# walaj/SeqLib

Hardware: AMD Instinct MI355X
Metric: aligned reads/sec (150 bp) via BWAAligner (higher is better)
Workload: dtype int32

## Files before the change

### seqlib_amd/csrc/dev_chain_coop.h

```cpp
#pragma once
#include "dev_chain.h"

__device__ __forceinline__ int64_t lane_read64(int64_t v, int src)
{
    const int s = __builtin_amdgcn_readfirstlane(src);
    const unsigned lo = (unsigned)__builtin_amdgcn_readlane((int)(v & 0xffffffffll), s);
    const unsigned hi = (unsigned)__builtin_amdgcn_readlane((int)(v >> 32), s);
    return (int64_t)(((unsigned long long)hi << 32) | lo);
}

struct CoopTables {
    int64_t *s_pos;
    int *s_ord;
    int *s_w, *s_cb, *s_ce, *s_first, *s_kept;
    signed char *s_kf;
};

template <typename I, int NCMAX, bool FINAL>
__device__ __noinline__ void dev_chain_read_coop(const DevFM<I> &fm, const DevRef &R, const Chunk &ck, const slx_opt &opt, int r, const CoopTables &T, int lane,
                                                 int nc_limit)
{
    int64_t *s_pos = T.s_pos; int *s_ord = T.s_ord, *s_w = T.s_w, *s_cb = T.s_cb, *s_ce = T.s_ce, *s_first = T.s_first, *s_kept = T.s_kept;
    signed char *s_kf = T.s_kf;
    {
        ReadWS w = make_ws(ck, r);
        const int len = (int)(ck.offs[r + 1] - ck.offs[r]);
        const int n_intv = (int)ck.intv_n[r];
        const qp_t *iinfo = (const qp_t *)ck.intv_info + (size_t)r * ck.cap_intv;
        const I *ix0 = (const I *)ck.intv_x0 + (size_t)r * ck.cap_intv;
        const I *ix2 = (const I *)ck.intv_x2 + (size_t)r * ck.cap_intv;
        int ns = 0, nc = 0;
        bool dup = false;
        KbTree kb;
        bool tree = false;
        int *l_tail = s_w, *l_lastql = s_cb, *l_lastoff = s_ce, *l_firstql = s_first, *l_rid = s_kept;
        const bool cnt16 = ck.seed_off[r + 1] - ck.seed_off[r] < 65536;
        for (int i = 0; i < n_intv; ++i) {
            const int qbeg = QP_HI(iinfo[i]), slen = QP_LO(iinfo[i]) - qbeg;
            const I x0 = ix0[i], x2 = ix2[i];
            const I step = x2 > (I)opt.max_occ ? x2 / (I)opt.max_occ : (I)1;
            I cm = (x2 + step - 1) / step;
            if (cm > (I)opt.max_occ) cm = (I)opt.max_occ;
            const int count_max = (int)cm;
            for (int base = 0; base < count_max; base += 64) {
                const int t = base + lane;
                const bool valid = t < count_max;
                int64_t rb_l = 0; int rid_l = -1;
                if (valid) {
                    rb_l = intv_pos<I>(fm, x0, (I)t * step);
                    rid_l = dev_intv2rid(R, rb_l, rb_l + slen);
                }
                const int nb = count_max - base < 64 ? count_max - base : 64;
                for (int u = 0; u < nb; ++u) {
                    const int rid = __builtin_amdgcn_readlane(rid_l, __builtin_amdgcn_readfirstlane(u));
                    if (rid < 0) continue;
                    const int64_t rbeg = lane_read64(rb_l, u);
                    int lo = -1, lower_c = -1;
                    bool to_add = true;
                    if (nc) {
                        if (tree) lower_c = kb.lower(rbeg);
                        else {
                            int b = 0, e = nc;
                            while (b < e) { const int m = (b + e) >> 1; if (s_pos[m] < rbeg) b = m + 1; else e = m; }
                            if (b == nc) lo = nc - 1;
                            else lo = rbeg < s_pos[b] ? b - 1 : b;
                            lower_c = lo >= 0 ? s_ord[lo] : -1;
                        }
                        if (lower_c >= 0) {
                            const int c = lower_c;
                            const int last = l_tail[c];
#ifdef SLX_WIDE
                            const qp_t lql = w.s_ql[last];
                            const int f_qbeg = w.s_qbeg(w.c_head[c]);
#else
                            const uint32_t lql = (uint32_t)l_lastql[c], fql = (uint32_t)l_firstql[c];
                            const int f_qbeg = (int)(fql >> 16);
#endif
                            const int l_qbeg = QP_HI(lql), l_len = QP_LO(lql);
                            const int64_t f_rbeg = tree ? w.c_pos[c] : s_pos[lo];
                            const int64_t l_rbeg = f_rbeg + l_lastoff[c];
                            const int64_t qend = l_qbeg + l_len, rend = l_rbeg + l_len;
                            int res;
                            if (rid != l_rid[c]) res = 0;
                            else if (qbeg >= f_qbeg && qbeg + slen <= qend && rbeg >= f_rbeg && rbeg + slen <= rend) res = 1;
                            else if ((l_rbeg < R.l_pac || f_rbeg < R.l_pac) && rbeg >= R.l_pac) res = 0;
                            else {
                                const int64_t x = qbeg - l_qbeg, y = rbeg - l_rbeg;
                                if (y >= 0 && x - y <= opt.w && y - x <= opt.w && x - l_len < opt.max_chain_gap && y - l_len < opt.max_chain_gap) {
                                    const int s = ns++;
                                    w.s_rbeg[s] = rbeg; w.s_ql[s] = QP_PACK(qbeg, slen); w.s_next[s] = -1; if (w.s_score) w.s_score[s] = slen;
                                    w.s_next[last] = s; w.c_tail[c] = s;
#ifdef SLX_WIDE
                                    w.c_n[c] = w.c_n[c] + 1;
                                    l_tail[c] = s; l_lastoff[c] = (int)(rbeg - f_rbeg);
#else
                                    if (cnt16) { l_firstql[c] = (int)(fql + 1u); w.c_n[c] = (int)(fql & 0xffff) + 1; }
                                    else w.c_n[c] = w.c_n[c] + 1;
                                    l_tail[c] = s; l_lastql[c] = (int)(((uint32_t)qbeg << 16) | (uint32_t)slen); l_lastoff[c] = (int)(rbeg - f_rbeg);
#endif
                                    res = 1;
                                } else res = 0;
                            }
                            to_add = !res;
                        }
                    }
                    if (to_add && !tree && lo >= 0 && s_pos[lo] == rbeg) dup = true;
                    if (to_add && dup && !tree && nc >= 2 * KB_T - 1) {
                        kb.mem = (int *)w.regs; kb.n_nodes = 0; kb.root = kb.alloc(0);
                        for (int h = 0; h < nc; ++h) kb.put(w.c_pos[h], h);
                        tree = true;
                    }
                    if (to_add && nc == nc_limit) {
                        if (FINAL) { if (lane == 0) dev_chain_read<I>(fm, R, ck, opt, r); }
                        else if (lane == 0) ck.n_chain[r] = -2;
                        return;
                    }
                    if (to_add) {
                        const int s = ns++, c = nc;
                        w.s_rbeg[s] = rbeg; w.s_ql[s] = QP_PACK(qbeg, slen); w.s_next[s] = -1; if (w.s_score) w.s_score[s] = slen;
                        w.c_pos[c] = rbeg; w.c_head[c] = s; w.c_tail[c] = s; w.c_n[c] = 1; w.c_rid[c] = rid;
#ifdef SLX_WIDE
                        l_tail[c] = s; l_lastoff[c] = 0; l_rid[c] = rid;
#else
                        l_tail[c] = s; l_lastql[c] = (int)(((uint32_t)qbeg << 16) | (uint32_t)slen); l_firstql[c] = (int)(((uint32_t)qbeg << 16) | 1u); l_lastoff[c] = 0; l_rid[c] = rid;
#endif
                        if (tree) kb.put(rbeg, c);
                        else {
                            for (int hi = nc; hi > lo + 1; hi -= 64) {
                                const int idx = hi - 1 - lane;
                                const bool mv = idx >= lo + 1;
                                int vo = 0; int64_t vp = 0;
                                if (mv) { vo = s_ord[idx]; vp = s_pos[idx]; }
                                if (mv) { s_ord[idx + 1] = vo; s_pos[idx + 1] = vp; }
                            }
                            s_ord[lo + 1] = c; s_pos[lo + 1] = rbeg;
                        }
                        ++nc;
                    }
                }
            }
        }
        if (tree) kb.traverse(s_ord);
        ck.frac_rep[r] = (float)ck.l_rep[r] / len;
        for (int c = lane; c < nc; c += 64) {
            const int wt = dev_chain_weight(w, c);
            s_w[c] = wt;
            s_cb[c] = w.s_qbeg(w.c_head[c]);
            s_ce[c] = w.s_qbeg(w.c_tail[c]) + w.s_len(w.c_tail[c]);
            s_first[c] = -1; s_kf[c] = 0;
        }
        int n_chn = 0;
        for (int base = 0; base < nc; base += 64) {
            const int m = base + lane;
            int c = 0; bool keep = false;
            if (m < nc) { c = s_ord[m]; keep = s_w[c] >= opt.min_chain_weight; }
            const unsigned long long bal = __ballot(keep);
            const int rank = __popcll(bal & ((1ull << lane) - 1ull));
            if (keep) s_ord[n_chn + rank] = c;
            n_chn += __popcll(bal);
        }
        int n_out = 0;
        if (n_chn > 0) {
            int *a = s_ord;
            ks_introsort_idx(n_chn, a, [&](int x, int y) { return s_w[x] > s_w[y]; });
            int n_kept = 0;
            s_kf[a[0]] = 3;
            s_kept[n_kept++] = 0;
            for (int i = 1; i < n_chn; ++i) {
                const int ci = a[i];
                const int bi = s_cb[ci], ei = s_ce[ci], wi = s_w[ci], li = ei - bi;
                const bool i_alt = ref_is_alt(R, w.c_rid[ci]) != 0;
                int large_ovlp = 0;
                bool broke = false;
                for (int kb = 0; kb < n_kept && !broke; kb += 64) {
                    const int k = kb + lane;
                    bool large = false, drop = false;
                    int cj = 0;
                    if (k < n_kept) {
                        cj = a[s_kept[k]];
                        const int bj = s_cb[cj], ej = s_ce[cj];
                        const int b_max = bj > bi ? bj : bi, e_min = ej < ei ? ej : ei;
                        if (e_min > b_max && (!ref_is_alt(R, w.c_rid[cj]) || i_alt)) {
                            const int lj = ej - bj;
                            const int min_l = li < lj ? li : lj;
                            if ((float)(e_min - b_max) >= (float)min_l * opt.mask_level && min_l < opt.max_chain_gap) {
                                large = true;
                                const int wj = s_w[cj];
                                if ((float)wi < (float)wj * opt.drop_ratio && wj - wi >= opt.min_seed_len << 1) drop = true;
                            }
                        }
                    }
                    const unsigned long long bd = __ballot(drop);
                    const int first_drop = bd ? (int)__ffsll((long long)bd) - 1 : 64;
                    const bool eff = large && lane <= first_drop;
                    if (eff && s_first[cj] < 0) s_first[cj] = i;
                    if (__ballot(eff)) large_ovlp = 1;
                    if (bd) broke = true;
                }
                if (!broke) { s_kept[n_kept++] = i; s_kf[ci] = large_ovlp ? 2 : 3; }
            }
            for (int i = lane; i < n_kept; i += 64) {
                const int c = a[s_kept[i]];
                if (s_first[c] >= 0) s_kf[a[s_first[c]]] = 1;
            }
            int i, k;
            for (i = k = 0; i < n_chn; ++i) {
                const int kf = s_kf[a[i]];
                if (kf == 0 || kf == 3) continue;
                if (++k >= opt.max_chain_extend) break;
            }
            for (int m = i + lane; m < n_chn; m += 64) if (s_kf[a[m]] < 3) s_kf[a[m]] = 0;
            for (int base = 0; base < n_chn; base += 64) {
                const int m = base + lane;
                int c = 0; bool keep = false;
                if (m < n_chn) { c = a[m]; keep = s_kf[c] != 0; }
                const unsigned long long bal = __ballot(keep);
                const int rank = __popcll(bal & ((1ull << lane) - 1ull));
                if (keep) w.ia[n_out + rank] = c;
                n_out += __popcll(bal);
            }
        }
        {
            int carry = 0;
            for (int base = 0; base < n_out; base += 64) {
                const int x = base + lane;
                const int c = x < n_out ? w.ia[x] : 0;
                const int cn = x < n_out ? w.c_n[c] : 0;
                int incl = cn;
                for (int d = 1; d < 64; d <<= 1) { const int t = __shfl_up(incl, d, 64); if (lane >= d) incl += t; }
                if (x < n_out) {
                    int off = carry + incl - cn;
                    w.c_first[c] = off;
                    for (int s = w.c_head[c]; s >= 0; s = w.s_next[s]) w.c_w[off++] = s;
                }
                carry += __shfl(incl, 63, 64);
            }
        }
        if (lane == 0) ck.n_chain[r] = n_out;
    }
}

template <typename I, int NCMAX, bool FINAL>
__global__ void __launch_bounds__(64) k_chain_coop(DevFM<I> fm, DevRef R, Chunk ck, DevOpt dopt, const int *order, unsigned int *queue,
                                                   const unsigned int *n_slots, int nc_limit)
{
    __shared__ int64_t s_pos[NCMAX + 64];
    __shared__ int s_ord[NCMAX + 64];
    __shared__ int s_w[NCMAX], s_cb[NCMAX], s_ce[NCMAX], s_first[NCMAX], s_kept[NCMAX];
    __shared__ signed char s_kf[NCMAX];
    CoopTables T;
    T.s_pos = s_pos; T.s_ord = s_ord; T.s_w = s_w; T.s_cb = s_cb; T.s_ce = s_ce; T.s_first = s_first; T.s_kept = s_kept; T.s_kf = s_kf;
    const int lane = threadIdx.x;
    const int n_todo = __builtin_amdgcn_readfirstlane((int)*n_slots);
    for (;;) {
        const int slot = (int)wave_take(queue, 1u);
        if (slot >= n_todo) break;
        const int r = order ? order[slot] : slot;
        const bool mine = !FINAL || __builtin_amdgcn_readfirstlane(ck.n_chain[r]) == -2;
        if (mine) dev_chain_read_coop<I, NCMAX, FINAL>(fm, R, ck, dopt.o, r, T, lane, nc_limit < NCMAX ? nc_limit : NCMAX);
    }
}
```

### seqlib_amd/csrc/dev_cig_band.h

```cpp
#pragma once
#include "dev_fin2.h"

template <int CPB, typename QF, typename TF>
__device__ int wave_ksw_global2_bandn(int qlen_, QF qf, int tlen_, TF tf, const slx_opt &o, int w_, uint8_t *z, int n_col_, int lane)
{
    const int qlen = __builtin_amdgcn_readfirstlane(qlen_), tlen = __builtin_amdgcn_readfirstlane(tlen_);
    const int w = __builtin_amdgcn_readfirstlane(w_), n_col = __builtin_amdgcn_readfirstlane(n_col_);
    const int o_del = o.o_del, e_del = o.e_del, o_ins = o.o_ins, e_ins = o.e_ins;
    const int oe_del = o_del + e_del, oe_ins = o_ins + e_ins;
    const MatCols mc = make_matcols(o.mat);
    auto pack_of = [&](int j) -> uint32_t {
        const int q = j >= 0 && j < qlen ? qf(j) : 4;
        return q == 0 ? mc.c[0] : q == 1 ? mc.c[1] : q == 2 ? mc.c[2] : q == 3 ? mc.c[3] : mc.c[4];
    };
    const int b0 = lane * CPB;
    int H[CPB], E[CPB];
    uint32_t P[CPB];
#pragma unroll
    for (int c = 0; c < CPB; ++c) {
        const int j = b0 + c - w;
        P[c] = pack_of(j);
        H[c] = j == 0 ? 0 : (j > 0 && j <= qlen && j <= w ? -(o_ins + e_ins * j) : DEV_MINUS_INF);
        E[c] = DEV_MINUS_INF;
    }
    int q_blk = (w + 1) >> 6;
    uint32_t q_cur = pack_of(q_blk * WAVE + lane), q_next = pack_of((q_blk + 1) * WAVE + lane);
    int tb_cur = lane < tlen ? tf(lane) : 0;
    int tb_next = WAVE + lane < tlen ? tf(WAVE + lane) : 0;
#pragma unroll 1
    for (int i = 0; i < tlen; ++i) {
        if ((i & (WAVE - 1)) == 0 && i) { tb_cur = tb_next; tb_next = i + WAVE + lane < tlen ? tf(i + WAVE + lane) : 0; }
        const int t = lane_read(tb_cur, i & (WAVE - 1));
        const uint32_t sh = (uint32_t)t << 3;
        const int beg = i > w ? i - w : 0;
        const int end = i + w + 1 < qlen ? i + w + 1 : qlen;
        const int b_lo = beg - (i - w), b_hi = end - (i - w);
        int m[CPB], exl[CPB];
        bool act[CPB];
        int run = G_NEG;
#pragma unroll
        for (int c = 0; c < CPB; ++c) {
            const int b = b0 + c;
            act[c] = b >= b_lo && b < b_hi;
            m[c] = H[c] + __builtin_amdgcn_sbfe((int)P[c], sh, 8u);
            exl[c] = run;
            const int u = act[c] ? m[c] - oe_ins + b * e_ins : G_NEG;
            run = imax(run, u);
        }
        const int incl = dpp_incl_max_scan_g(run);
        const int lane_ex = dpp_get<0x138, 0xf, 0xf>(G_NEG, incl);
        int e2v[CPB];
#pragma unroll
        for (int c = 0; c < CPB; ++c) {
            const int b = b0 + c;
            const int ex = imax(lane_ex, exl[c]);
            int f = DEV_MINUS_INF - (b - b_lo) * e_ins;
            if (b > b_lo) f = imax(f, ex - (b - 1) * e_ins);
            const int e = E[c];
            int d = m[c] >= e ? 0 : 1;
            int hh = m[c] >= e ? m[c] : e;
            d = hh >= f ? d : 2;
            hh = hh >= f ? hh : f;
            int tt = m[c] - oe_del;
            int e2 = e - e_del;
            d |= e2 > tt ? 1 << 2 : 0;
            e2 = e2 > tt ? e2 : tt;
            tt = m[c] - oe_ins;
            const int f2 = f - e_ins;
            d |= f2 > tt ? 2 << 4 : 0;
            if (act[c] && z) z[(size_t)i * n_col + (b - b_lo)] = (uint8_t)d;
            if (act[c]) H[c] = hh;
            if (b == w - (i + 1)) H[c] = -(o_del + e_del * (i + 1));
            e2v[c] = act[c] ? e2 : DEV_MINUS_INF;
        }
        const int e_in = dpp_get<0x130, 0xf, 0xf>(DEV_MINUS_INF, e2v[0]);
        const uint32_t p_in = (uint32_t)dpp_get<0x130, 0xf, 0xf>(0, (int)P[0]);
        const int jn = i + 1 + w;
        if ((jn >> 6) != q_blk) { q_blk = jn >> 6; q_cur = q_next; q_next = pack_of((q_blk + 1) * WAVE + lane); }
        const uint32_t p_new = jn < qlen ? (uint32_t)lane_read((int)q_cur, jn & (WAVE - 1)) : mc.c[4];
#pragma unroll
        for (int c = 0; c < CPB; ++c) {
            E[c] = c + 1 < CPB ? e2v[c + 1 < CPB ? c + 1 : c] : e_in;
            const uint32_t p_up = c + 1 < CPB ? P[c + 1 < CPB ? c + 1 : c] : p_in;
            P[c] = (b0 + c) == 2 * w ? p_new : p_up;
        }
    }
    const int bf = qlen - 1 - (tlen - 1 - w);
    const int src = bf / CPB, kk = bf - src * CPB;
    int pick = H[0];
#pragma unroll
    for (int c = 1; c < CPB; ++c) pick = kk == c ? H[c] : pick;
    return lane_read(pick, src);
}

#define GB_THREADS 256
#define GB_WAVES (GB_THREADS / WAVE)
struct GbShared { int scan[2][GB_WAVES], edge[2][GB_WAVES]; int result; };

enum { GI_START = 0, GI_NEUTRAL = 1, GI_LOAD = 2 };
struct GRun {
    int i0 = 0, i1 = 0;
    int init = GI_START;
    int rec_row = -1;
    const int *win_in = nullptr;
    int *win_rec = nullptr, *win_out = nullptr;
    int pick = -1;
};

template <int CPB, typename QF, typename TF>
__device__ void block_gband_rows(int qlen, QF qf, int tlen, TF tf, const slx_opt &o, int w, uint8_t *z, int n_col, GbShared &S, const GRun &run)
{
    constexpr int NB = GB_THREADS * CPB;
    const int tid = threadIdx.x, lane = tid & (WAVE - 1), wv = tid >> 6;
    const int o_del = o.o_del, e_del = o.e_del, o_ins = o.o_ins, e_ins = o.e_ins;
    const int oe_del = o_del + e_del, oe_ins = o_ins + e_ins;
    const MatCols mc = make_matcols(o.mat);
    auto pack_of = [&](int j) -> uint32_t {
        const int q = j >= 0 && j < qlen ? qf(j) : 4;
        return q == 0 ? mc.c[0] : q == 1 ? mc.c[1] : q == 2 ? mc.c[2] : q == 3 ? mc.c[3] : mc.c[4];
    };
    const int i0 = run.i0, i1 = run.i1 < tlen ? run.i1 : tlen;
    const int b0 = tid * CPB;
    int H[CPB], E[CPB];
    uint32_t P[CPB];
#pragma unroll
    for (int c = 0; c < CPB; ++c) {
        const int j = i0 + b0 + c - w;
        P[c] = pack_of(j);
        if (run.init == GI_START) { H[c] = j == 0 ? 0 : (j > 0 && j <= qlen && j <= w ? -(o_ins + e_ins * j) : DEV_MINUS_INF); E[c] = DEV_MINUS_INF; }
        else if (run.init == GI_NEUTRAL) { H[c] = 0; E[c] = DEV_MINUS_INF; }
        else { H[c] = run.win_in[b0 + c]; E[c] = run.win_in[NB + b0 + c]; }
    }
    const int top = (wv + 1) * WAVE * CPB;
    int q_blk = (i0 + top - w) >> 6;
    uint32_t q_cur = pack_of(q_blk * WAVE + lane), q_next = pack_of((q_blk + 1) * WAVE + lane);
    const int tb0 = i0 & ~(WAVE - 1);
    int tb_cur = tb0 + lane < tlen ? tf(tb0 + lane) : 0;
    int tb_next = tb0 + WAVE + lane < tlen ? tf(tb0 + WAVE + lane) : 0;
    __syncthreads();
#pragma unroll 1
    for (int i = i0; i < i1; ++i) {
        const int par = i & 1;
        if ((i & (WAVE - 1)) == 0 && i > i0) { tb_cur = tb_next; tb_next = i + WAVE + lane < tlen ? tf(i + WAVE + lane) : 0; }
        const int t = lane_read(tb_cur, i & (WAVE - 1));
        const uint32_t sh = (uint32_t)t << 3;
        const int beg = i > w ? i - w : 0;
        const int end = i + w + 1 < qlen ? i + w + 1 : qlen;
        const int b_lo = beg - (i - w), b_hi = end - (i - w);
        int m[CPB], exl[CPB];
        bool act[CPB];
        int run_u = G_NEG;
#pragma unroll
        for (int c = 0; c < CPB; ++c) {
            const int b = b0 + c;
            act[c] = b >= b_lo && b < b_hi;
            m[c] = H[c] + __builtin_amdgcn_sbfe((int)P[c], sh, 8u);
            exl[c] = run_u;
            const int u = act[c] ? m[c] - oe_ins + b * e_ins : G_NEG;
            run_u = imax(run_u, u);
        }
        const int incl = dpp_incl_max_scan_g(run_u);
        int lane_ex = dpp_get<0x138, 0xf, 0xf>(G_NEG, incl);
        if (lane == WAVE - 1) S.scan[par][wv] = incl;
        __syncthreads();
        if (i > i0 && lane == WAVE - 1 && wv < GB_WAVES - 1) E[CPB - 1] = S.edge[par ^ 1][wv + 1];
        if (i == run.rec_row) {
#pragma unroll
            for (int c = 0; c < CPB; ++c) { run.win_rec[b0 + c] = H[c]; run.win_rec[NB + b0 + c] = E[c]; }
        }
        uint8_t *zr = (z && i >= run.rec_row) ? z : nullptr;
#pragma unroll
        for (int k = 0; k < GB_WAVES - 1; ++k) { const int v = S.scan[par][k]; if (k < wv) lane_ex = imax(lane_ex, v); }
        int e2v[CPB];
#pragma unroll
        for (int c = 0; c < CPB; ++c) {
            const int b = b0 + c;
            const int ex = imax(lane_ex, exl[c]);
            int f = DEV_MINUS_INF - (b - b_lo) * e_ins;
            if (b > b_lo) f = imax(f, ex - (b - 1) * e_ins);
            const int e = E[c];
            int d = m[c] >= e ? 0 : 1;
            int hh = m[c] >= e ? m[c] : e;
            d = hh >= f ? d : 2;
            hh = hh >= f ? hh : f;
            int tt = m[c] - oe_del;
            int e2 = e - e_del;
            d |= e2 > tt ? 1 << 2 : 0;
            e2 = e2 > tt ? e2 : tt;
            tt = m[c] - oe_ins;
            const int f2 = f - e_ins;
            d |= f2 > tt ? 2 << 4 : 0;
            if (act[c] && zr) zr[(size_t)i * n_col + (b - b_lo)] = (uint8_t)d;
            if (act[c]) H[c] = hh;
            if (b == w - (i + 1)) H[c] = -(o_del + e_del * (i + 1));
            e2v[c] = act[c] ? e2 : DEV_MINUS_INF;
        }
        if (lane == 0) S.edge[par][wv] = e2v[0];
        const int e_in = dpp_get<0x130, 0xf, 0xf>(DEV_MINUS_INF, e2v[0]);
        const uint32_t p_in = (uint32_t)dpp_get<0x130, 0xf, 0xf>(0, (int)P[0]);
        const int jn = i - w + top;
        if ((jn >> 6) != q_blk) { q_blk = jn >> 6; q_cur = q_next; q_next = pack_of((q_blk + 1) * WAVE + lane); }
        const uint32_t p_top = (uint32_t)lane_read((int)q_cur, jn & (WAVE - 1));
#pragma unroll
        for (int c = 0; c < CPB; ++c) {
            E[c] = c + 1 < CPB ? e2v[c + 1 < CPB ? c + 1 : c] : e_in;
            const uint32_t p_up = c + 1 < CPB ? P[c + 1 < CPB ? c + 1 : c] : p_in;
            P[c] = (c == CPB - 1 && lane == WAVE - 1) ? p_top : p_up;
        }
    }
    if (run.win_out) {
        __syncthreads();
        if (i1 > i0 && lane == WAVE - 1 && wv < GB_WAVES - 1) E[CPB - 1] = S.edge[(i1 - 1) & 1][wv + 1];
#pragma unroll
        for (int c = 0; c < CPB; ++c) { run.win_out[b0 + c] = H[c]; run.win_out[NB + b0 + c] = E[c]; }
    }
    if (run.pick >= 0) {
#pragma unroll
        for (int c = 0; c < CPB; ++c) if (b0 + c == run.pick) S.result = H[c];
        __syncthreads();
    }
}

template <int CPB, typename QF, typename TF>
__device__ int block_ksw_global2_bandn(int qlen, QF qf, int tlen, TF tf, const slx_opt &o, int w, uint8_t *z, int n_col, GbShared &S)
{
    GRun run;
    run.i0 = 0; run.i1 = tlen; run.init = GI_START;
    run.pick = qlen - 1 - (tlen - 1 - w);
    block_gband_rows<CPB>(qlen, qf, tlen, tf, o, w, z, n_col, S, run);
    return S.result;
}

#define CIG_BAND_MAX_COLS (13 * WAVE)

struct CigBlockShared { GbShared gb; unsigned long long off; int n_ops_dummy; };
struct GJob;
struct GPlan;
struct CigSeg { const GPlan *P = nullptr; const GJob *gj = nullptr; unsigned int job_t = 0; int *scratch = nullptr; };
template <typename QF, typename TF>
__device__ int gseg_join_any(int lq, QF qf, int rlen, TF tf, const slx_opt &o, const CigSeg &cs, uint8_t *z, GbShared &S);
__device__ bool gseg_is_cut(const CigSeg &cs, int ww, int n_col, unsigned long long *z_off);

template <bool BLOCK>
static __device__ __noinline__ bool dev_cig_band_job(const DevRef &R, const Chunk &ck, const slx_opt &opt, const FinLists &fl, uint32_t slot, int lane, CigBlockShared *SB = nullptr,
                                                     const CigSeg *cs = nullptr)
{
    [[maybe_unused]] const bool wave0 = !BLOCK || threadIdx.x < WAVE;
    const DJob j = fl.jobs[slot];
    DHit h = ck.hits[slot];
    const uint8_t *query = ck.codes + ck.offs[j.r];
    const int l_query = (int)(ck.offs[j.r + 1] - ck.offs[j.r]);
    const int lq = j.qe - j.qb;
    const int64_t rb = j.rb, re = j.re;
    const uint8_t *qseg = query + j.qb;
    const bool valid = !(lq <= 0 || rb >= re || (rb < R.l_pac && re > R.l_pac));
    const int rlen = (int)(re - rb);
    const bool rev = rb >= R.l_pac;
    auto qf = [&](int x) { return (int)(rev ? qseg[lq - 1 - x] : qseg[x]); };
    auto tf = [&](int y) { return rev ? ref_base(R, re - 1 - y) : ref_base(R, rb + y); };
    int w2 = j.w2, score = 0, last_sc = -(1 << 30), w_used = 0, n_col = 0;
    uint8_t *z = nullptr;
    if (valid) {
        for (int it = 0; it < 3; ++it) {
            w2 = w2 < opt.w << 2 ? w2 : opt.w << 2;
            int ww, max_gap, max_ins, max_del, min_w;
            max_ins = (int)((double)(((lq + 1) >> 1) * opt.mat[0] - opt.o_ins) / opt.e_ins + 1.);
            max_del = (int)((double)(((lq + 1) >> 1) * opt.mat[0] - opt.o_del) / opt.e_del + 1.);
            max_gap = max_ins > max_del ? max_ins : max_del;
            max_gap = max_gap > 1 ? max_gap : 1;
            const int dl = rlen - lq < 0 ? lq - rlen : rlen - lq;
            ww = (max_gap + dl + 1) >> 1;
            ww = ww < w2 ? ww : w2;
            min_w = dl + 3;
            ww = ww > min_w ? ww : min_w;
            w_used = ww;
            n_col = lq < 2 * ww + 1 ? lq : 2 * ww + 1;
            if (2 * ww + 1 > CIG_BAND_MAX_COLS) return false;
            const unsigned long long need = (unsigned long long)n_col * (unsigned long long)rlen;
            unsigned long long off = 0;
            if constexpr (BLOCK) {
                unsigned long long z_off = 0;
                if (it == 0 && cs && gseg_is_cut(*cs, ww, n_col, &z_off)) {
                    z = ck.zarena + z_off;
                    score = gseg_join_any(lq, qf, rlen, tf, opt, *cs, z, SB->gb);
                    if (score == last_sc || w2 == opt.w << 2) break;
                    last_sc = score;
                    w2 <<= 1;
                    if (!(score < j.truesc - opt.a)) break;
                    continue;
                }
                __syncthreads();
                if (block_tid() == 0) SB->off = atomicAdd(ck.zused, need);
                __syncthreads();
                off = SB->off;
            } else off = wave_take_u64(ck.zused, need);
            if (off + need > ck.zcap) { if (lane == 0 && wave0) atomicOr(ck.flags, OVF_ZARENA | (BLOCK ? OVS_Z_BAND_BLOCK : OVS_Z_BAND)); return true; }
            z = ck.zarena + off;
            const int cols = 2 * ww + 1;
            if constexpr (BLOCK) {
                if (cols <= GB_THREADS) score = block_ksw_global2_bandn<1>(lq, qf, rlen, tf, opt, ww, z, n_col, SB->gb);
                else if (cols <= 2 * GB_THREADS) score = block_ksw_global2_bandn<2>(lq, qf, rlen, tf, opt, ww, z, n_col, SB->gb);
                else score = block_ksw_global2_bandn<4>(lq, qf, rlen, tf, opt, ww, z, n_col, SB->gb);
            } else
            if (cols <= WAVE) score = wave_ksw_global2_bandn<1>(lq, qf, rlen, tf, opt, ww, z, n_col, lane);
            else if (cols <= 2 * WAVE) score = wave_ksw_global2_bandn<2>(lq, qf, rlen, tf, opt, ww, z, n_col, lane);
            else if (cols <= 4 * WAVE) score = wave_ksw_global2_bandn<4>(lq, qf, rlen, tf, opt, ww, z, n_col, lane);
            else if (cols <= 8 * WAVE) score = wave_ksw_global2_bandn<8>(lq, qf, rlen, tf, opt, ww, z, n_col, lane);
            else score = wave_ksw_global2_bandn<13>(lq, qf, rlen, tf, opt, ww, z, n_col, lane);
            if (score == last_sc || w2 == opt.w << 2) break;
            last_sc = score;
            w2 <<= 1;
            if (!(score < j.truesc - opt.a)) break;
        }
    }
    if constexpr (BLOCK) {
        __threadfence();
        __syncthreads();
        if (!wave0) return true;
    }
    int n_ops = 0;
    if (valid) {
        __threadfence();
        dev_traceback_wave(z, n_col, lq, rlen, w_used, lane, [&](int, int) { ++n_ops; });
    }
    n_ops = __builtin_amdgcn_readfirstlane(n_ops);
    const unsigned long long need = (unsigned long long)n_ops + 2;
    const unsigned long long base = wave_take_u64(ck.cigused, need);
    if (base + need > ck.cigcap) { if (lane == 0) atomicOr(ck.flags, OVF_CIGAR | OVS_C_BAND); return true; }
    uint32_t *cg = ck.cigpool + base + 1;
    if (valid) {
        int wp = n_ops;
        dev_traceback_wave(z, n_col, lq, rlen, w_used, lane, [&](int op, int len) { cg[--wp] = (uint32_t)len << 4 | (uint32_t)op; });
        int x = 0, y = 0, n_mm = 0, n_gap = 0;
        for (int k = 0; k < n_ops; ++k) {
            const uint32_t cw = cg[k];
            const int op = (int)(cw & 0xf), len = (int)(cw >> 4);
            if (op == 0) {
                for (int u = lane; u < len; u += WAVE) n_mm += qf(x + u) != tf(y + u);
                x += len; y += len;
            } else if (op == 2) { if (k > 0 && k < n_ops - 1) n_gap += len; y += len; }
            else if (op == 1) { x += len; n_gap += len; }
        }
        for (int d = 32; d >= 1; d >>= 1) n_mm += __shfl_xor(n_mm, d, WAVE);
        h.nm = n_mm + n_gap;
    }
    dev_finish_hit(R, ck, j, l_query, h, (int64_t)base + 1, n_ops);
    if (lane == 0) ck.hits[slot] = h;
    return true;
}

__global__ void __launch_bounds__(64) k_cig_band(DevRef R, Chunk ck, DevOpt dopt, FinLists fl, uint32_t *rest, unsigned int *n_rest)
{
    const int lane = threadIdx.x;
    const unsigned int n_jobs = *fl.n_dp;
    for (;;) {
        const unsigned int t = wave_take(fl.q_dp, 1u);
        if (t >= n_jobs) break;
        const uint32_t slot = fl.dp_list[t];
        if (!dev_cig_band_job<false>(R, ck, dopt.o, fl, slot, lane) && lane == 0) rest[atomicAdd(n_rest, 1u)] = slot;
    }
}


struct RegsBlockShared {
    GbShared gb;
    int cmd, w, l_query, rlen, rev;
    const uint8_t *qseg;
    int64_t rb, re;
};

__device__ __noinline__ int regs_block_dp(const DevRef &R, const slx_opt &o, RegsBlockShared &S)
{
    const int w = S.w, l_query = S.l_query, rlen = S.rlen;
    const bool rev = S.rev != 0;
    const uint8_t *qseg = S.qseg;
    const int64_t rb = S.rb, re = S.re;
    auto qf = [&](int x) { return (int)(rev ? qseg[l_query - 1 - x] : qseg[x]); };
    auto tf = [&](int y) { return rev ? ref_base(R, re - 1 - y) : ref_base(R, rb + y); };
    const int cols = 2 * w + 1;
    if (cols <= GB_THREADS) return block_ksw_global2_bandn<1>(l_query, qf, rlen, tf, o, w, nullptr, 0, S.gb);
    if (cols <= 2 * GB_THREADS) return block_ksw_global2_bandn<2>(l_query, qf, rlen, tf, o, w, nullptr, 0, S.gb);
    return block_ksw_global2_bandn<4>(l_query, qf, rlen, tf, o, w, nullptr, 0, S.gb);
}

struct PMemo { const GJob *jobs; const int *off, *n; };
__device__ bool pseg_lookup(const PMemo *pm, int r, int w_arg, unsigned long long q_off, int l_query, int64_t rb, int64_t re, int *score);

#ifdef PSEG_DEBUG
__device__ void pseg_debug_miss(const PMemo *pm, int r, int w_arg, unsigned long long q_off, int l_query, int64_t rb, int64_t re);
#endif
struct WaveScorerLong {
    const DevRef &R; const slx_opt &o; const Chunk &ck; int lane; int *eh_h, *eh_e;
    RegsBlockShared *SB;
    const PMemo *pm = nullptr;
    const int *cur_r = nullptr;
    __device__ int operator()(int w_, int l_query, const uint8_t *qseg, int64_t rb, int64_t re) const
    {
        if (l_query <= 0 || rb >= re || (rb < R.l_pac && re > R.l_pac)) return 0;
        if (pm) { int ms = 0; if (pseg_lookup(pm, *cur_r, w_, (unsigned long long)(qseg - ck.codes), l_query, rb, re, &ms)) return ms; }
#ifdef PSEG_DEBUG
        if (pm && lane == 0 && re - rb >= 16384) pseg_debug_miss(pm, *cur_r, w_, (unsigned long long)(qseg - ck.codes), l_query, rb, re);
#endif
        const int rlen = (int)(re - rb);
        const bool rev = rb >= R.l_pac;
        auto qf = [&](int x) { return (int)(rev ? qseg[l_query - 1 - x] : qseg[x]); };
        auto tf = [&](int y) { return rev ? ref_base(R, re - 1 - y) : ref_base(R, rb + y); };
        if (l_query == rlen && w_ == 0) {
            int sc = 0;
            for (int i = lane; i < l_query; i += WAVE) sc += o.mat[tf(i) * 5 + qf(i)];
            for (int d = 32; d >= 1; d >>= 1) sc += __shfl_xor(sc, d, WAVE);
            return sc;
        }
        int max_ins = (int)((double)(((l_query + 1) >> 1) * o.mat[0] - o.o_ins) / o.e_ins + 1.);
        int max_del = (int)((double)(((l_query + 1) >> 1) * o.mat[0] - o.o_del) / o.e_del + 1.);
        int max_gap = max_ins > max_del ? max_ins : max_del;
        max_gap = max_gap > 1 ? max_gap : 1;
        const int dl = rlen - l_query < 0 ? l_query - rlen : rlen - l_query;
        int w = (max_gap + dl + 1) >> 1;
        w = w < w_ ? w : w_;
        const int min_w = dl + 3;
        w = w > min_w ? w : min_w;
        const int cols = 2 * w + 1;
        if (SB && cols > 2 * WAVE && cols <= 4 * GB_THREADS && rlen >= 2048) {
            if (lane == 0) { SB->w = w; SB->l_query = l_query; SB->rlen = rlen; SB->rev = rev ? 1 : 0; SB->qseg = qseg; SB->rb = rb; SB->re = re; SB->cmd = 1; }
            __syncthreads();
            return regs_block_dp(R, o, *SB);
        }
        if (cols <= WAVE) return wave_ksw_global2_bandn<1>(l_query, qf, rlen, tf, o, w, nullptr, 0, lane);
        if (cols <= 2 * WAVE) return wave_ksw_global2_bandn<2>(l_query, qf, rlen, tf, o, w, nullptr, 0, lane);
        if (cols <= 4 * WAVE) return wave_ksw_global2_bandn<4>(l_query, qf, rlen, tf, o, w, nullptr, 0, lane);
        if (cols <= 8 * WAVE) return wave_ksw_global2_bandn<8>(l_query, qf, rlen, tf, o, w, nullptr, 0, lane);
        if (cols <= CIG_BAND_MAX_COLS) return wave_ksw_global2_bandn<13>(l_query, qf, rlen, tf, o, w, nullptr, 0, lane);
        int sc = 0;
        if (lane == 0) sc = dev_gen_cigar2<0>(R, o, ck, w_, l_query, qseg, rb, re, false, eh_h, eh_e).score;
        return lane_read(sc, 0);
    }
};

template <int MAXQ, int NB>
__global__ void __launch_bounds__(GB_THREADS) k_regs_wave_long(DevRef R, Chunk ck, DevOpt dopt, FinLists fl, const int *order, unsigned int *queue, const unsigned int *n_slots,
                                                               PMemo pm)
{
    __shared__ int s_idx[NB], s_ka[NB], s_kb[NB], s_qe[NB], s_rid[NB], s_w[NB];
    __shared__ int64_t s_k64[NB], s_rb[NB];
    __shared__ RegsBlockShared SB;
    if ((int)blockIdx.x * WAVE >= ck.long_threads) return;
    if (threadIdx.x >= WAVE) {
        for (;;) {
            __syncthreads();
            if (SB.cmd == 0) break;
            regs_block_dp(R, dopt.o, SB);
        }
        return;
    }
    const int lane = threadIdx.x;
    SortStage ss;
    ss.idx = s_idx; ss.k64 = s_k64; ss.ka = s_ka; ss.kb = s_kb; ss.m_rb = s_rb; ss.m_qe = s_qe; ss.m_rid = s_rid; ss.m_w = s_w;
    ss.nmax = NB; ss.lane = lane;
    int *eh_h = ck.long_scratch + (size_t)blockIdx.x * WAVE * 2 * ck.long_stride, *eh_e = eh_h + ck.long_stride;
    int cur_r = 0;
    WaveScorerLong sc{R, dopt.o, ck, lane, eh_h, eh_e, &SB, pm.jobs ? &pm : nullptr, &cur_r};
    const int n_todo = __builtin_amdgcn_readfirstlane((int)*n_slots);
    for (;;) {
        const int slot = (int)wave_take(queue, 1u);
        if (slot >= n_todo) break;
        const int r = order ? order[slot] : slot;
        cur_r = r;
        dev_regs_read<MAXQ>(R, ck, dopt.o, fl, r, sc, lane == 0, &ss);
    }
    if (lane == 0) SB.cmd = 0;
    __syncthreads();
}
```

### seqlib_amd/csrc/dev_fin.h

```cpp
#pragma once
#include "dev_ext.h"

#define DEV_MINUS_INF (-0x40000000)

template <typename QF, typename TF>
__device__ int dev_ksw_global2(int qlen, QF qf, int tlen, TF tf, const slx_opt &o, int w, uint8_t *z, int n_col, int *eh_h, int *eh_e)
{
    const int8_t *mat = o.mat;
    const int o_del = o.o_del, e_del = o.e_del, o_ins = o.o_ins, e_ins = o.e_ins;
    const int oe_del = o_del + e_del, oe_ins = o_ins + e_ins;
    int i, j;
    eh_h[0] = 0; eh_e[0] = DEV_MINUS_INF;
    for (j = 1; j <= qlen && j <= w; ++j) { eh_h[j] = -(o_ins + e_ins * j); eh_e[j] = DEV_MINUS_INF; }
    for (; j <= qlen; ++j) eh_h[j] = eh_e[j] = DEV_MINUS_INF;
    for (i = 0; i < tlen; ++i) {
        int f = DEV_MINUS_INF, h1, beg, end, t;
        const int8_t *qrow = mat + tf(i) * 5;
        beg = i > w ? i - w : 0;
        end = i + w + 1 < qlen ? i + w + 1 : qlen;
        h1 = beg == 0 ? -(o_del + e_del * (i + 1)) : DEV_MINUS_INF;
        uint8_t *zi = z ? z + (size_t)i * n_col : nullptr;
        for (j = beg; j < end; ++j) {
            int h, m = eh_h[j], e = eh_e[j];
            uint8_t d;
            eh_h[j] = h1;
            m += qrow[qf(j)];
            d = m >= e ? 0 : 1;
            h = m >= e ? m : e;
            d = h >= f ? d : 2;
            h = h >= f ? h : f;
            h1 = h;
            t = m - oe_del;
            e -= e_del;
            d |= e > t ? 1 << 2 : 0;
            e = e > t ? e : t;
            eh_e[j] = e;
            t = m - oe_ins;
            f -= e_ins;
            d |= f > t ? 2 << 4 : 0;
            f = f > t ? f : t;
            if (zi) zi[j - beg] = d;
        }
        eh_h[end] = h1; eh_e[end] = DEV_MINUS_INF;
    }
    return eh_h[qlen];
}

template <typename ZAT, typename F>
__device__ void dev_traceback_at(ZAT zat, int qlen, int tlen, int w, F emit)
{
    int i = tlen - 1, k = (i + w + 1 < qlen ? i + w + 1 : qlen) - 1, which = 0;
    int cur_op = -1, cur_len = 0;
    auto unit = [&](int op, int len) {
        if (op == cur_op) cur_len += len;
        else { if (cur_op >= 0) emit(cur_op, cur_len); cur_op = op; cur_len = len; }
    };
    while (i >= 0 && k >= 0) {
        which = zat(i, k - (i > w ? i - w : 0)) >> (which << 1) & 3;
        if (which == 0) { unit(0, 1); --i; --k; }
        else if (which == 1) { unit(2, 1); --i; }
        else { unit(1, 1); --k; }
    }
    if (i >= 0) unit(2, i + 1);
    if (k >= 0) unit(1, k + 1);
    if (cur_op >= 0) emit(cur_op, cur_len);
}
template <typename F>
__device__ void dev_traceback(const uint8_t *z, int n_col, int qlen, int tlen, int w, F emit)
{
    dev_traceback_at([&](int i, int c) { return (int)z[(size_t)i * n_col + c]; }, qlen, tlen, w, emit);
}

struct GenCig {
    int score;
    bool valid;
    bool fast;
    bool rev;
    int w, n_col, qlen, tlen;
    uint8_t *z;
};

template <int MAXQ>
__device__ GenCig dev_gen_cigar2(const DevRef &R, const slx_opt &o, const Chunk &ck, int w_, int l_query, const uint8_t *qseg,
                                 int64_t rb, int64_t re, bool want_z, int *eh_h, int *eh_e)
{
    GenCig g;
    g.score = 0; g.valid = false; g.fast = false; g.rev = false; g.w = 0; g.n_col = 0; g.qlen = l_query; g.tlen = 0; g.z = nullptr;
    if (l_query <= 0 || rb >= re || (rb < R.l_pac && re > R.l_pac)) return g;
    g.valid = true;
    const int rlen = (int)(re - rb);
    g.tlen = rlen;
    g.rev = rb >= R.l_pac;
    const bool rev = g.rev;
    auto qf = [&](int j) { return (int)(rev ? qseg[l_query - 1 - j] : qseg[j]); };
    auto tf = [&](int i) { return rev ? ref_base(R, re - 1 - i) : ref_base(R, rb + i); };
    if (l_query == rlen && w_ == 0) {
        g.fast = true;
        int sc = 0;
        for (int i = 0; i < l_query; ++i) sc += o.mat[tf(i) * 5 + qf(i)];
        g.score = sc;
    } else {
        int w, max_gap, max_ins, max_del, min_w;
        max_ins = (int)((double)(((l_query + 1) >> 1) * o.mat[0] - o.o_ins) / o.e_ins + 1.);
        max_del = (int)((double)(((l_query + 1) >> 1) * o.mat[0] - o.o_del) / o.e_del + 1.);
        max_gap = max_ins > max_del ? max_ins : max_del;
        max_gap = max_gap > 1 ? max_gap : 1;
        const int dl = rlen - l_query < 0 ? l_query - rlen : rlen - l_query;
        w = (max_gap + dl + 1) >> 1;
        w = w < w_ ? w : w_;
        min_w = dl + 3;
        w = w > min_w ? w : min_w;
        g.w = w;
        g.n_col = l_query < 2 * w + 1 ? l_query : 2 * w + 1;
        if (want_z) {
            const unsigned long long need = (unsigned long long)g.n_col * (unsigned long long)rlen;
            const unsigned long long off = atomicAdd(ck.zused, need);
            if (off + need > ck.zcap) { atomicOr(ck.flags, OVF_ZARENA | OVS_Z_GEN); g.valid = false; return g; }
            g.z = ck.zarena + off;
        }
        g.score = dev_ksw_global2(l_query, qf, rlen, tf, o, w, g.z, g.n_col, eh_h, eh_e);
    }
    return g;
}

__device__ __forceinline__ int dev_patch_pre(const DevRef &R, const slx_opt &o, int64_t a_rb, int64_t a_re, int a_qb, int a_qe, int a_w,
                                             int64_t b_rb, int64_t b_re, int b_qb, int b_qe, int b_w)
{
    int w;
    double r;
    if (a_rb < R.l_pac && b_rb >= R.l_pac) return -1;
    if (a_qb >= b_qb || a_qe >= b_qe || a_re >= b_re) return -1;
    w = (int)((a_re - b_rb) - (a_qe - b_qb));
    w = w > 0 ? w : -w;
    r = (double)(a_re - b_rb) / (double)(b_re - a_rb) - (double)(a_qe - b_qb) / (double)(b_qe - a_qb);
    r = r > 0. ? r : -r;
    if (a_re < b_rb || a_qe < b_qb) {
        if (w > o.w << 1 || r >= (double)0.05f) return -1;
    } else if (w > o.w << 2 || r >= (double)(0.05f * 2)) return -1;
    w += a_w + b_w;
    w = w < o.w << 2 ? w : o.w << 2;
    return w;
}

template <int MAXQ, typename SC>
__device__ int dev_patch_reg(const DevRef &R, const slx_opt &o, const Chunk &ck, const uint8_t *query, const DReg &a, const DReg &b,
                             int *_w, SC &sc)
{
    int score, q_s, r_s;
    const int w = dev_patch_pre(R, o, a.rb, a.re, a.qb, a.qe, a.w, b.rb, b.re, b.qb, b.qe, b.w);
    if (w < 0) return 0;
    score = sc(w, b.qe - a.qb, query + a.qb, a.rb, b.re);
    q_s = (int)((double)(b.qe - a.qb) / (double)((b.qe - b.qb) + (a.qe - a.qb)) * (double)(b.score + a.score) + .499);
    r_s = (int)((double)(b.re - a.rb) / (double)((b.re - b.rb) + (a.re - a.rb)) * (double)(b.score + a.score) + .499);
    if ((double)score / (double)(q_s > r_s ? q_s : r_s) < (double)0.90f) return 0;
    *_w = w;
    return score;
}

__device__ __forceinline__ uint64_t dev_hash_64(uint64_t key)
{
    key += ~(key << 32); key ^= (key >> 22); key += ~(key << 13); key ^= (key >> 8);
    key += (key << 3); key ^= (key >> 15); key += ~(key << 27); key ^= (key >> 31);
    return key;
}

__device__ __forceinline__ uint64_t dev_lrand48_nth(uint64_t state, uint64_t n)
{
    const uint64_t M = (1ULL << 48) - 1;
    uint64_t a = 0x5DEECE66DULL, c = 0xBULL, ra = 1, rc = 0;
    while (n) {
        if (n & 1) { ra = (ra * a) & M; rc = (rc * a + c) & M; }
        c = ((a + 1) * c) & M;
        a = (a * a) & M;
        n >>= 1;
    }
    return ((ra * (state & M) + rc) & M) >> 17;
}

__device__ __forceinline__ int dev_infer_bw(int l1, int l2, int score, int a, int q, int r)
{
    int w;
    if (l1 == l2 && l1 * a - score < (q + r - a) << 1) return 0;
    w = (int)((double)((l1 < l2 ? l1 : l2) * a - score - q) / r + 2.);
    const int d = l1 - l2 < 0 ? l2 - l1 : l1 - l2;
    if (w < d) w = d;
    return w;
}

__device__ inline int dev_approx_mapq_se(const slx_opt &o, const DReg &a, const Chunk &ck)
{
    int mapq, l, sub = a.sub ? a.sub : o.min_seed_len * o.a;
    double identity;
    sub = a.csub > sub ? a.csub : sub;
    if (sub >= a.score) return 0;
    l = a.qe - a.qb > a.re - a.rb ? a.qe - a.qb : (int)(a.re - a.rb);
    identity = 1. - (double)(l * o.a - a.score) / (double)(o.a + o.b) / (double)l;
    if (a.score == 0) mapq = 0;
    else if (o.mapQ_coef_len > 0) {
        double tmp;
        if ((float)l < o.mapQ_coef_len) tmp = 1.;
        else {
            if (l >= ck.log_lut_n) { atomicOr(ck.flags, ERR_LOGLUT); return 0; }
            tmp = (double)o.mapQ_coef_fac / ck.log_lut[l];
        }
        tmp *= identity * identity;
        mapq = (int)(6.02 * (double)(a.score - sub) / (double)o.a * tmp * tmp + .499);
    } else {
        if (a.seedcov >= ck.log_lut_n || a.seedcov < 1) { atomicOr(ck.flags, ERR_LOGLUT); return 0; }
        mapq = (int)(30.0 * (1. - (double)sub / (double)a.score) * ck.log_lut[a.seedcov] + .499);
        mapq = identity < 0.95 ? (int)((double)mapq * identity * identity + .499) : mapq;
    }
    if (a.sub_n > 0) {
        if (a.sub_n + 1 >= ck.log_lut_n) { atomicOr(ck.flags, ERR_LOGLUT); return 0; }
        mapq -= (int)(4.343 * ck.log_lut[a.sub_n + 1] + .499);
    }
    if (mapq > 60) mapq = 60;
    if (mapq < 0) mapq = 0;
    mapq = (int)((double)mapq * (1. - (double)a.frac_rep) + .499);
    return mapq;
}

__device__ inline void dev_mark_primary_alt(const DevRef &R, const slx_opt &opt, const ReadWS &w, int n, uint64_t id)
{
    int *a = w.ia, *z = w.ib;
    int *par = (int *)w.srt;
    DReg *G = w.regs;
    auto alt = [&](int h) { return ref_is_alt(R, G[h].rid); };
    int tmp = opt.a + opt.b;
    tmp = opt.o_del + opt.e_del > tmp ? opt.o_del + opt.e_del : tmp;
    tmp = opt.o_ins + opt.e_ins > tmp ? opt.o_ins + opt.e_ins : tmp;
    auto core = [&](int m) {
        int nz = 0;
        z[nz++] = 0;
        for (int i = 1; i < m; ++i) {
            int k;
            DReg &ai = G[a[i]];
            for (k = 0; k < nz; ++k) {
                DReg &aj = G[a[z[k]]];
                const int b_max = aj.qb > ai.qb ? aj.qb : ai.qb;
                const int e_min = aj.qe < ai.qe ? aj.qe : ai.qe;
                if (e_min > b_max) {
                    const int min_l = ai.qe - ai.qb < aj.qe - aj.qb ? ai.qe - ai.qb : aj.qe - aj.qb;
                    if ((float)(e_min - b_max) >= (float)min_l * opt.mask_level) {
                        if (aj.sub == 0) aj.sub = ai.score;
                        if (aj.score - ai.score <= tmp && (alt(a[z[k]]) || !alt(a[i]))) ++aj.sub_n;
                        break;
                    }
                }
            }
            if (k == nz) z[nz++] = i;
            else ai.secondary = z[k];
        }
    };
    int n_pri = 0;
    for (int i = 0; i < n; ++i) {
        DReg &p = G[a[i]];
        p.sub = 0; p.secondary = -1;
        p.hash = dev_hash_64(id + (uint64_t)i);
        if (!alt(a[i])) ++n_pri;
    }
    ks_introsort_idx(n, a, [&](int x, int y) {
        const DReg &X = G[x], &Y = G[y];
        if (X.score != Y.score) return X.score > Y.score;
        const int ax = alt(x), ay = alt(y);
        return ax < ay || (ax == ay && X.hash < Y.hash);
    });
    core(n);
    if (n_pri < n) {
        for (int i = 0; i < n; ++i) { const int sidx = G[a[i]].secondary; par[a[i]] = sidx >= 0 ? a[sidx] : -1; }
        if (n_pri > 0)
            ks_introsort_idx(n, a, [&](int x, int y) {
                const DReg &X = G[x], &Y = G[y];
                const int ax = alt(x), ay = alt(y);
                if (ax != ay) return ax < ay;
                return X.score > Y.score || (X.score == Y.score && X.hash < Y.hash);
            });
        for (int i = 0; i < n; ++i) z[a[i]] = i;
        for (int i = 0; i < n; ++i) {
            const int h = a[i], ph = par[h];
            if (ph >= 0) { par[h] = z[ph]; if (alt(h)) G[h].secondary = 0x7fffffff; }
            else par[h] = -1;
        }
        if (n_pri > 0) {
            for (int i = 0; i < n_pri; ++i) { DReg &p = G[a[i]]; p.sub = 0; p.secondary = -1; }
            core(n_pri);
        }
    } else
        for (int i = 0; i < n; ++i) par[a[i]] = G[a[i]].secondary;
}

struct SortStage {
    int *idx;
    int64_t *k64;
    int *ka, *kb;
    int64_t *m_rb;
    int *m_qe, *m_rid, *m_w;
    int nmax;
    int lane;
};

template <int MAXQ>
__device__ __forceinline__ void fin_sync()
{
    if constexpr (MAXQ > 704) { __builtin_amdgcn_fence(__ATOMIC_ACQ_REL, "workgroup"); __builtin_amdgcn_wave_barrier(); }
    else __syncthreads();
}

template <int MAXQ, typename SC>
__device__ int dev_fin_regs(const DevRef &R, const Chunk &ck, const slx_opt &opt, ReadWS &w, int r, const uint8_t *query, int l_query, SC &sc,
                            const SortStage *ss = nullptr, bool *defer = nullptr)
{
        int n = ck.n_reg[r];
        int *a = w.ia;
        DReg *G = w.regs;
        const bool staged = ss != nullptr && n <= ss->nmax && n >= 2;
        const bool dbg = ck.dbg_cyc && ck.dbg_stage == 2;
        unsigned long long t0 = dbg ? __builtin_readcyclecounter() : 0ull, t1 = t0, t2 = t0, t3 = t0;
        auto sort_handles = [&](int m, auto fill, auto less_lds, auto less_glb) {
            if (!staged) { ks_introsort_idx(m, a, less_glb); return; }
            __threadfence_block();
            for (int i = ss->lane; i < m; i += 64) { const int h = a[i]; ss->idx[i] = h; fill(h); }
            fin_sync<MAXQ>();
            bool tie = m > 768;
            if (!tie) for (int e = ss->lane; e < m; e += 64) {
                const int he = ss->idx[e];
                int rank = 0;
                for (int j = 0; j < m; ++j) {
                    const int hj = ss->idx[j];
                    const bool lt = less_lds(hj, he);
                    rank += lt ? 1 : 0;
                    if (!lt && j != e && !less_lds(he, hj)) tie = true;
                }
                ss->m_w[e] = rank;
            }
            if (!__any(tie)) {
                fin_sync<MAXQ>();
                for (int e = ss->lane; e < m; e += 64) ss->m_rid[ss->m_w[e]] = ss->idx[e];
                fin_sync<MAXQ>();
                for (int e = ss->lane; e < m; e += 64) { const int h = ss->m_rid[e]; ss->idx[e] = h; a[e] = h; }
            } else {
                fin_sync<MAXQ>();
                if (ss->lane == 0) ks_introsort_idx(m, ss->idx, less_lds);
                fin_sync<MAXQ>();
                for (int i = ss->lane; i < m; i += 64) a[i] = ss->idx[i];
            }
            fin_sync<MAXQ>();
            __threadfence_block();
        };
        if (staged) { for (int i = ss->lane; i < n; i += 64) a[i] = i; __threadfence_block(); }
        else for (int i = 0; i < n; ++i) a[i] = i;
        if (n > 1) {
            sort_handles(n, [&](int h) { ss->k64[h] = G[h].re; },
                         [&](int x, int y) { return ss->k64[x] < ss->k64[y]; },
                         [&](int x, int y) { return G[x].re < G[y].re; });
            if (dbg) t1 = __builtin_readcyclecounter();
            if (defer && !staged && n <= 64) {
                for (int i = 1; i < n; ++i) {
                    const DReg &p = G[a[i]];
                    if (p.rid != G[a[i - 1]].rid || p.rb >= G[a[i - 1]].re + opt.max_chain_gap) continue;
                    for (int j = i - 1; j >= 0 && p.rid == G[a[j]].rid && p.rb < G[a[j]].re + opt.max_chain_gap; --j) {
                        const DReg &q = G[a[j]];
                        if (q.rb < p.rb && dev_patch_pre(R, opt, q.rb, q.re, q.qb, q.qe, q.w, p.rb, p.re, p.qb, p.qe, p.w) >= 0) { *defer = true; return -1; }
                    }
                }
            }
            if (staged) { for (int i = ss->lane; i < n; i += 64) G[i].n_comp = 1; __threadfence_block(); }
            else for (int i = 0; i < n; ++i) G[a[i]].n_comp = 1;
            if (staged) {
                const int lane = ss->lane;
                int64_t *m_re = ss->k64; int *m_sc = ss->ka, *m_qb = ss->kb;
                for (int h = lane; h < n; h += 64) {
                    const DReg &g = G[h];
                    ss->m_rb[h] = g.rb; m_re[h] = g.re; m_qb[h] = g.qb; ss->m_qe[h] = g.qe; ss->m_rid[h] = g.rid; m_sc[h] = g.score; ss->m_w[h] = g.w;
                }
                fin_sync<MAXQ>();
                for (int i = 1; i < n; ++i) {
                    const int ph = ss->idx[i], prevh = ss->idx[i - 1];
                    if (ss->m_rid[ph] != ss->m_rid[prevh] || ss->m_rb[ph] >= m_re[prevh] + opt.max_chain_gap) continue;
                    int jtop = i - 1;
                    while (jtop >= 0) {
                        const int64_t p_rb = ss->m_rb[ph], p_re = m_re[ph];
                        const int p_qb = m_qb[ph], p_qe = ss->m_qe[ph], p_rid = ss->m_rid[ph], p_sc = m_sc[ph], p_w = ss->m_w[ph];
                        const int j = jtop - lane;
                        const bool valid = j >= 0;
                        const int qh = ss->idx[valid ? j : 0];
                        const int64_t q_rb = ss->m_rb[qh], q_re = m_re[qh];
                        const int q_qb = m_qb[qh], q_qe = ss->m_qe[qh], q_sc = m_sc[qh], q_w = ss->m_w[qh];
                        const bool cond = valid && p_rid == ss->m_rid[qh] && p_rb < q_re + opt.max_chain_gap;
                        const unsigned long long stopm = __ballot(!cond);
                        const int first_stop = stopm ? (int)__ffsll((long long)stopm) - 1 : 64;
                        const bool live = lane < first_stop;
                        int cat = 0;
                        if (live && q_qe != q_qb) {
                            const int64_t orr = q_re - p_rb;
                            const int64_t oq = q_qb < p_qb ? q_qe - p_qb : p_qe - q_qb;
                            const int64_t mr = q_re - q_rb < p_re - p_rb ? q_re - q_rb : p_re - p_rb;
                            const int64_t mq = q_qe - q_qb < p_qe - p_qb ? q_qe - q_qb : p_qe - p_qb;
                            if ((float)orr > opt.mask_level_redun * (float)mr && (float)oq > opt.mask_level_redun * (float)mq) cat = p_sc < q_sc ? 2 : 1;
                            else if (q_rb < p_rb && dev_patch_pre(R, opt, q_rb, q_re, q_qb, q_qe, q_w, p_rb, p_re, p_qb, p_qe, p_w) >= 0) cat = 3;
                        }
                        const unsigned long long evm = __ballot(cat >= 2);
                        const int first_ev = evm ? (int)__ffsll((long long)evm) - 1 : 64;
                        if (cat == 1 && lane < first_ev) { ss->m_qe[qh] = q_qb; G[qh].qe = q_qb; }
                        fin_sync<MAXQ>();
                        if (first_ev == 64) {
                            if (first_stop < 64) break;
                            jtop -= 64;
                            continue;
                        }
                        const int ev_cat = __builtin_amdgcn_readlane(cat, first_ev);
                        const int ev_q = __builtin_amdgcn_readlane(qh, first_ev);
                        if (ev_cat == 2) {
                            if (lane == 0) { ss->m_qe[ph] = p_qb; G[ph].qe = p_qb; }
                            fin_sync<MAXQ>();
                            break;
                        }
                        {
                            DReg &pp = G[ph];
                            DReg &q = G[ev_q];
                            int ww = 0;
                            const int score = dev_patch_reg<MAXQ>(R, opt, ck, query, q, pp, &ww, sc);
                            if (score > 0) {
                                pp.n_comp += q.n_comp + 1;
                                pp.seedcov = pp.seedcov > q.seedcov ? pp.seedcov : q.seedcov;
                                pp.sub = pp.sub > q.sub ? pp.sub : q.sub;
                                pp.csub = pp.csub > q.csub ? pp.csub : q.csub;
                                pp.qb = q.qb; pp.rb = q.rb;
                                pp.truesc = pp.score = score;
                                pp.w = ww;
                                q.qb = q.qe;
                                if (lane == 0) {
                                    m_qb[ph] = m_qb[ev_q]; ss->m_rb[ph] = ss->m_rb[ev_q]; m_sc[ph] = score; ss->m_w[ph] = ww;
                                    m_qb[ev_q] = ss->m_qe[ev_q];
                                }
                                fin_sync<MAXQ>();
                            }
                        }
                        jtop -= first_ev + 1;
                    }
                }
                __threadfence_block();
            } else
            for (int i = 1; i < n; ++i) {
                DReg &p = G[a[i]];
                if (p.rid != G[a[i - 1]].rid || p.rb >= G[a[i - 1]].re + opt.max_chain_gap) continue;
                for (int j = i - 1; j >= 0 && p.rid == G[a[j]].rid && p.rb < G[a[j]].re + opt.max_chain_gap; --j) {
                    DReg &q = G[a[j]];
                    int64_t orr, oq, mr, mq;
                    int score, ww;
                    if (q.qe == q.qb) continue;
                    orr = q.re - p.rb;
                    oq = q.qb < p.qb ? q.qe - p.qb : p.qe - q.qb;
                    mr = q.re - q.rb < p.re - p.rb ? q.re - q.rb : p.re - p.rb;
                    mq = q.qe - q.qb < p.qe - p.qb ? q.qe - q.qb : p.qe - p.qb;
                    if ((float)orr > opt.mask_level_redun * (float)mr && (float)oq > opt.mask_level_redun * (float)mq) {
                        if (p.score < q.score) { p.qe = p.qb; break; }
                        else q.qe = q.qb;
                    } else if (q.rb < p.rb && (score = dev_patch_reg<MAXQ>(R, opt, ck, query, q, p, &ww, sc)) > 0) {
                        p.n_comp += q.n_comp + 1;
                        p.seedcov = p.seedcov > q.seedcov ? p.seedcov : q.seedcov;
                        p.sub = p.sub > q.sub ? p.sub : q.sub;
                        p.csub = p.csub > q.csub ? p.csub : q.csub;
                        p.qb = q.qb; p.rb = q.rb;
                        p.truesc = p.score = score;
                        p.w = ww;
                        q.qb = q.qe;
                    }
                }
            }
            if (dbg) t2 = __builtin_readcyclecounter();
            auto compact_staged = [&](int n_in, int first_forced) {
                int m = 0;
                for (int base = 0; base < n_in; base += 64) {
                    const int i = base + ss->lane;
                    const int h = i < n_in ? ss->idx[i] : 0;
                    const bool keep = i < n_in && (i < first_forced || ss->m_qe[h] > ss->kb[h]);
                    const unsigned long long km = __ballot(keep);
                    const int pos = m + (int)__builtin_amdgcn_mbcnt_hi((uint32_t)(km >> 32), __builtin_amdgcn_mbcnt_lo((uint32_t)km, 0u));
                    if (keep) a[pos] = h;
                    m += (int)__popcll(km);
                }
                __threadfence_block();
                return m;
            };
            int m = 0;
            if (staged) m = compact_staged(n, 0);
            else for (int i = 0; i < n; ++i) if (G[a[i]].qe > G[a[i]].qb) a[m++] = a[i];
            n = m;
            sort_handles(n, [&](int h) { ss->ka[h] = G[h].score; ss->k64[h] = G[h].rb; ss->kb[h] = G[h].qb; },
                         [&](int x, int y) {
                             const int sx = ss->ka[x], sy = ss->ka[y];
                             const int64_t bx = ss->k64[x], by = ss->k64[y];
                             return sx > sy || (sx == sy && (bx < by || (bx == by && ss->kb[x] < ss->kb[y])));
                         },
                         [&](int x, int y) {
                             const DReg &X = G[x], &Y = G[y];
                             return X.score > Y.score || (X.score == Y.score && (X.rb < Y.rb || (X.rb == Y.rb && X.qb < Y.qb)));
                         });
            if (staged) {
                for (int i = 1 + ss->lane; i < n; i += 64) {
                    const int h = ss->idx[i], hp = ss->idx[i - 1];
                    if (ss->ka[h] == ss->ka[hp] && ss->k64[h] == ss->k64[hp] && ss->kb[h] == ss->kb[hp]) { G[h].qe = ss->kb[h]; ss->m_qe[h] = ss->kb[h]; }
                }
                fin_sync<MAXQ>();
                n = compact_staged(n, 1);
            } else {
                for (int i = 1; i < n; ++i)
                    if (G[a[i]].score == G[a[i - 1]].score && G[a[i]].rb == G[a[i - 1]].rb && G[a[i]].qb == G[a[i - 1]].qb)
                        G[a[i]].qe = G[a[i]].qb;
                m = n > 0 ? 1 : 0;
                for (int i = 1; i < n; ++i) if (G[a[i]].qe > G[a[i]].qb) a[m++] = a[i];
                n = m;
            }
        }
        if (dbg) t3 = __builtin_readcyclecounter();
        ck.na[r] = n;
        if (n > 0) {
            const uint64_t id = dev_lrand48_nth(ck.rng_state, ck.first_ordinal + (uint64_t)r + 1);
            int tmp = opt.a + opt.b;
            tmp = opt.o_del + opt.e_del > tmp ? opt.o_del + opt.e_del : tmp;
            tmp = opt.o_ins + opt.e_ins > tmp ? opt.o_ins + opt.e_ins : tmp;
            auto core_staged = [&](int m, const int *l_alt) {
                const int lane = ss->lane;
                int *l_sub = ss->m_rid, *l_subn = ss->m_w, *l_sec = (int *)ss->k64, *l_z = (int *)ss->k64 + ss->nmax;
                fin_sync<MAXQ>();
                for (int i = lane; i < m; i += 64) { const int h = ss->idx[i]; l_sub[h] = 0; l_subn[h] = G[h].sub_n; l_sec[h] = -1; }
                if (lane == 0) l_z[0] = 0;
                fin_sync<MAXQ>();
                int nz = 1;
                for (int i = 1; i < m; ++i) {
                    const int hi = ss->idx[i];
                    const int i_qb = ss->kb[hi], i_qe = ss->m_qe[hi], i_sc = ss->ka[hi];
                    int found = -1;
                    for (int kb0 = 0; kb0 < nz && found < 0; kb0 += 64) {
                        const int k = kb0 + lane;
                        bool hit = false;
                        if (k < nz) {
                            const int hj = ss->idx[l_z[k]];
                            const int j_qb = ss->kb[hj], j_qe = ss->m_qe[hj];
                            const int b_max = j_qb > i_qb ? j_qb : i_qb;
                            const int e_min = j_qe < i_qe ? j_qe : i_qe;
                            if (e_min > b_max) {
                                const int min_l = i_qe - i_qb < j_qe - j_qb ? i_qe - i_qb : j_qe - j_qb;
                                hit = (float)(e_min - b_max) >= (float)min_l * opt.mask_level;
                            }
                        }
                        const unsigned long long hm = __ballot(hit);
                        if (hm) found = kb0 + (int)__ffsll((long long)hm) - 1;
                    }
                    if (found >= 0) {
                        if (lane == 0) {
                            const int zi = l_z[found];
                            const int hj = ss->idx[zi];
                            if (l_sub[hj] == 0) l_sub[hj] = i_sc;
                            if (ss->ka[hj] - i_sc <= tmp && (!l_alt || l_alt[hj] || !l_alt[hi])) ++l_subn[hj];
                            l_sec[hi] = zi;
                        }
                    } else { if (lane == 0) l_z[nz] = i; ++nz; }
                    fin_sync<MAXQ>();
                }
                for (int i = lane; i < m; i += 64) { const int h = ss->idx[i]; DReg &p = G[h]; p.sub = l_sub[h]; p.sub_n = l_subn[h]; p.secondary = l_sec[h]; }
                __threadfence_block();
                fin_sync<MAXQ>();
            };
            if (R.ann_alt && staged) {
                const int lane = ss->lane;
                int *l_alt = (int *)ss->m_rb, *l_par = (int *)ss->m_rb + ss->nmax, *par = (int *)w.srt;
                fin_sync<MAXQ>();
                int n_pri = 0;
                for (int base = 0; base < n; base += 64) {
                    const int i = base + lane;
                    bool pri = false;
                    if (i < n) {
                        const int h = a[i];
                        DReg &p = G[h];
                        p.sub = 0; p.secondary = -1; p.hash = dev_hash_64(id + (uint64_t)i);
                        const int al = ref_is_alt(R, p.rid);
                        l_alt[h] = al;
                        pri = !al;
                    }
                    n_pri += (int)__popcll(__ballot(pri));
                }
                __threadfence_block();
                sort_handles(n, [&](int h) { ss->ka[h] = G[h].score; ss->k64[h] = (int64_t)G[h].hash; },
                             [&](int x, int y) {
                                 const int sx = ss->ka[x], sy = ss->ka[y];
                                 if (sx != sy) return sx > sy;
                                 const int ax = l_alt[x], ay = l_alt[y];
                                 return ax < ay || (ax == ay && (uint64_t)ss->k64[x] < (uint64_t)ss->k64[y]);
                             },
                             [&](int x, int y) { return false; });
                core_staged(n, l_alt);
                if (n_pri < n) {
                    for (int i = lane; i < n; i += 64) { const int h = ss->idx[i], sidx = G[h].secondary; l_par[h] = sidx >= 0 ? ss->idx[sidx] : -1; }
                    fin_sync<MAXQ>();
                    if (n_pri > 0)
                        sort_handles(n, [&](int h) { ss->ka[h] = G[h].score; ss->k64[h] = (int64_t)G[h].hash; },
                                     [&](int x, int y) {
                                         const int ax = l_alt[x], ay = l_alt[y];
                                         if (ax != ay) return ax < ay;
                                         const int sx = ss->ka[x], sy = ss->ka[y];
                                         return sx > sy || (sx == sy && (uint64_t)ss->k64[x] < (uint64_t)ss->k64[y]);
                                     },
                                     [&](int x, int y) { return false; });
                    int *l_rank = (int *)ss->k64;
                    fin_sync<MAXQ>();
                    for (int i = lane; i < n; i += 64) l_rank[ss->idx[i]] = i;
                    fin_sync<MAXQ>();
                    for (int i = lane; i < n; i += 64) {
                        const int h = ss->idx[i], ph = l_par[h];
                        if (ph >= 0) { par[h] = l_rank[ph]; if (l_alt[h]) G[h].secondary = 0x7fffffff; }
                        else par[h] = -1;
                    }
                    if (n_pri > 0) {
                        __threadfence_block();
                        core_staged(n_pri, l_alt);
                    }
                } else
                    for (int i = lane; i < n; i += 64) { const int h = ss->idx[i]; par[h] = G[h].secondary; }
                __threadfence_block();
                fin_sync<MAXQ>();
            } else if (R.ann_alt) {
                dev_mark_primary_alt(R, opt, w, n, id);
            } else {
            if (staged) {
                for (int i = ss->lane; i < n; i += 64) { DReg &p = G[a[i]]; p.sub = 0; p.secondary = -1; p.hash = dev_hash_64(id + (uint64_t)i); }
                __threadfence_block();
            } else for (int i = 0; i < n; ++i) {
                DReg &p = G[a[i]];
                p.sub = 0; p.secondary = -1;
                p.hash = dev_hash_64(id + (uint64_t)i);
            }
            sort_handles(n, [&](int h) { ss->ka[h] = G[h].score; ss->k64[h] = (int64_t)G[h].hash; },
                         [&](int x, int y) {
                             const int sx = ss->ka[x], sy = ss->ka[y];
                             return sx > sy || (sx == sy && (uint64_t)ss->k64[x] < (uint64_t)ss->k64[y]);
                         },
                         [&](int x, int y) {
                             const DReg &X = G[x], &Y = G[y];
                             return X.score > Y.score || (X.score == Y.score && X.hash < Y.hash);
                         });
            if (staged) core_staged(n, nullptr);
            else {
            int *z = w.ib, nz = 0;
            z[nz++] = 0;
            for (int i = 1; i < n; ++i) {
                int k;
                DReg &ai = G[a[i]];
                for (k = 0; k < nz; ++k) {
                    DReg &aj = G[a[z[k]]];
                    const int b_max = aj.qb > ai.qb ? aj.qb : ai.qb;
                    const int e_min = aj.qe < ai.qe ? aj.qe : ai.qe;
                    if (e_min > b_max) {
                        const int min_l = ai.qe - ai.qb < aj.qe - aj.qb ? ai.qe - ai.qb : aj.qe - aj.qb;
                        if ((float)(e_min - b_max) >= (float)min_l * opt.mask_level) {
                            if (aj.sub == 0) aj.sub = ai.score;
                            if (aj.score - ai.score <= tmp) ++aj.sub_n;
                            break;
                        }
                    }
                }
                if (k == nz) z[nz++] = i;
                else ai.secondary = z[k];
            }
            }
            }
        }
        if (dbg) {
            const unsigned long long t4 = __builtin_readcyclecounter();
            ck.dbg_cyc[r] = t4 - t0; ck.dbg_cyc[(size_t)ck.n_reads + r] = t1 - t0; ck.dbg_cyc[2 * (size_t)ck.n_reads + r] = t2 - t1;
            ck.dbg_cyc[3 * (size_t)ck.n_reads + r] = t3 - t2;
        }
        return n;
}


struct HitsSoA {
    int64_t *hit_off; int32_t *rid; int64_t *pos; uint16_t *flag; uint8_t *mapq; int32_t *score, *nm, *na, *n_cigar_ops;
    int64_t *cig_off; uint32_t *cigar;
    int32_t *xa_parent, *sub;
};

__global__ void k_hit_counts(Chunk ck, unsigned long long *n_cig_words)
{
    const int r = blockIdx.x * blockDim.x + threadIdx.x;
    if (r >= ck.n_reads) return;
    const uint64_t o = ck.seed_off[r];
    unsigned long long c = 0;
    for (int i = 0; i < ck.n_hit[r]; ++i) c += (unsigned long long)ck.hits[o + ck.ic[o + i]].n_cigar;
    n_cig_words[r] = c;
}

__global__ void k_compact(Chunk ck, const unsigned long long *hit_off, const unsigned long long *cig_off_read, HitsSoA out,
                          int64_t read_base, int64_t hit_base, int64_t cig_base)
{
    const int r = blockIdx.x * blockDim.x + threadIdx.x;
    if (r >= ck.n_reads) return;
    const uint64_t o = ck.seed_off[r];
    int64_t ho = hit_base + (int64_t)hit_off[r];
    int64_t co = cig_base + (int64_t)cig_off_read[r];
    out.hit_off[read_base + r] = ho;
    for (int i = 0; i < ck.n_hit[r]; ++i, ++ho) {
        const DHit &h = ck.hits[o + ck.ic[o + i]];
        out.rid[ho] = h.rid; out.pos[ho] = h.pos; out.flag[ho] = (uint16_t)h.flag; out.mapq[ho] = (uint8_t)h.mapq;
        if (out.xa_parent) {
            out.xa_parent[ho] = ((h.flag >> 16) & 0x7fff) - 1;
            const DReg &g = ck.regs[o + ck.ia[o + ck.ic[o + i]]];
            out.sub[ho] = h.flag < 0 ? (g.sub > g.csub ? g.sub : g.csub) : -1;
        }
        out.score[ho] = h.score; out.nm[ho] = h.nm; out.na[ho] = ck.na[r]; out.n_cigar_ops[ho] = h.n_cigar;
        out.cig_off[ho] = co;
        for (int k = 0; k < h.n_cigar; ++k) out.cigar[co++] = ck.cigpool[h.cig_start + k];
    }
}
```

### seqlib_amd/csrc/dev_fin2.h

```cpp
#pragma once
#include "dev_fin.h"
#include "dev_ext_reg.h"
#include "dev_nm8.h"

#ifndef LANE_CIG_BAND
#define LANE_CIG_BAND 33
#endif
#define LANE_CIG_MAXQ 158
#define LANE_CIG_MAXT 400
#define LANE_NEG (-16000)
#define LANE_FIN_LIMIT 8000
static_assert(LANE_NEG + LANE_FIN_LIMIT <= -LANE_FIN_LIMIT && LANE_NEG >= -32768 && LANE_FIN_LIMIT <= 32767, "16-bit cells of k_cig_lanes");
#define LANE_IL_WORDS(max_len) (((LANE_CIG_BAND + 3) / 4) * (((max_len) < LANE_CIG_MAXQ ? (max_len) : LANE_CIG_MAXQ) + 16))
struct alignas(8) DJob {
    int64_t rb, re;
    int qb, qe;
    int w2, truesc;
    int r, pad;
};

struct FinLists {
    DJob *jobs;
    uint32_t *fast_list, *dp_list;
    unsigned int *n_fast, *n_dp, *q_dp;
    uint32_t *lane_list;
    unsigned int *n_lane;
};

#define G_NEG ((int)0x80000000)

__device__ __forceinline__ int dpp_incl_max_scan_g(int v)
{
    v = imax(v, dpp_get<0x111, 0xf, 0xf>(G_NEG, v));
    v = imax(v, dpp_get<0x112, 0xf, 0xf>(G_NEG, v));
    v = imax(v, dpp_get<0x114, 0xf, 0xf>(G_NEG, v));
    v = imax(v, dpp_get<0x118, 0xf, 0xf>(G_NEG, v));
    v = imax(v, dpp_get<0x142, 0xa, 0xf>(G_NEG, v));
    v = imax(v, dpp_get<0x143, 0xc, 0xf>(G_NEG, v));
    return v;
}

template <int CPL, typename QF, typename TF>
__device__ int wave_ksw_global2(int qlen_, QF qf, int tlen_, TF tf, const slx_opt &o, const MatRows &mr, int w_, uint8_t *z, int n_col_, int lane)
{
    const int qlen = __builtin_amdgcn_readfirstlane(qlen_), tlen = __builtin_amdgcn_readfirstlane(tlen_);
    const int w = __builtin_amdgcn_readfirstlane(w_), n_col = __builtin_amdgcn_readfirstlane(n_col_);
    const int o_del = o.o_del, e_del = o.e_del, o_ins = o.o_ins, e_ins = o.e_ins;
    const int oe_del = o_del + e_del, oe_ins = o_ins + e_ins;
    const int j0 = lane * CPL;
    const MatCols mc = make_matcols(o.mat);
    int H[CPL], E[CPL];
    uint32_t P[CPL];
#pragma unroll
    for (int k = 0; k < CPL; ++k) {
        const int j = j0 + k;
        const int q = j < qlen ? qf(j) : 4;
        P[k] = q == 0 ? mc.c[0] : q == 1 ? mc.c[1] : q == 2 ? mc.c[2] : q == 3 ? mc.c[3] : mc.c[4];
        H[k] = j == 0 ? 0 : (j <= qlen && j <= w ? -(o_ins + e_ins * j) : DEV_MINUS_INF);
        E[k] = DEV_MINUS_INF;
    }
    int tb_cur = lane < tlen ? tf(lane) : 0;
    int tb_next = WAVE + lane < tlen ? tf(WAVE + lane) : 0;
#ifdef CIG_NOUNROLL
#pragma unroll 1
#endif
    for (int i = 0; i < tlen; ++i) {
        if ((i & (WAVE - 1)) == 0 && i) { tb_cur = tb_next; tb_next = i + WAVE + lane < tlen ? tf(i + WAVE + lane) : 0; }
        const int t = lane_read(tb_cur, i & (WAVE - 1));
        const uint32_t sh = (uint32_t)t << 3;
        const int beg = i > w ? i - w : 0;
        const int end = i + w + 1 < qlen ? i + w + 1 : qlen;
        const int h1_init = beg == 0 ? -(o_del + e_del * (i + 1)) : DEV_MINUS_INF;
        int M[CPL], pre[CPL], h[CPL];
        int run = G_NEG;
#pragma unroll
        for (int k = 0; k < CPL; ++k) {
            const int j = j0 + k;
            const bool act = j >= beg && j < end;
            const int s = __builtin_amdgcn_sbfe((int)P[k], sh, 8u);
            M[k] = H[k] + s;
            const int u = act ? M[k] - oe_ins + j * e_ins : G_NEG;
            run = imax(run, u);
            pre[k] = run;
        }
        const int incl = dpp_incl_max_scan_g(run);
        const int excl = dpp_get<0x138, 0xf, 0xf>(G_NEG, incl);
        uint8_t *zi = z ? z + (size_t)i * n_col : nullptr;
#pragma unroll
        for (int k = 0; k < CPL; ++k) {
            const int j = j0 + k;
            const bool act = j >= beg && j < end;
            const int ex = k == 0 ? excl : imax(excl, pre[k - 1]);
            int f = DEV_MINUS_INF - (j - beg) * e_ins;
            if (j > beg) f = imax(f, ex - (j - 1) * e_ins);
            const int m = M[k], e = E[k];
            int d = m >= e ? 0 : 1;
            int hh = m >= e ? m : e;
            d = hh >= f ? d : 2;
            hh = hh >= f ? hh : f;
            h[k] = hh;
            int tt = m - oe_del;
            int e2 = e - e_del;
            d |= e2 > tt ? 1 << 2 : 0;
            e2 = e2 > tt ? e2 : tt;
            tt = m - oe_ins;
            const int f2 = f - e_ins;
            d |= f2 > tt ? 2 << 4 : 0;
            if (act) { E[k] = e2; if (zi) zi[j - beg] = (uint8_t)d; }
        }
        const int h_left = dpp_get<0x138, 0xf, 0xf>(0, h[CPL - 1]);
#pragma unroll
        for (int k = 0; k < CPL; ++k) {
            const int j = j0 + k;
            const int hp = k == 0 ? h_left : h[k - 1];
            if (j - 1 >= beg && j - 1 < end) H[k] = hp;
            if (end > beg) { if (j == beg) H[k] = h1_init; if (j == end) E[k] = DEV_MINUS_INF; }
            else if (j == end) { H[k] = h1_init; E[k] = DEV_MINUS_INF; }
        }
    }
    const int src = qlen / CPL, kk = qlen - src * CPL;
    int pick = H[0];
#pragma unroll
    for (int k = 1; k < CPL; ++k) pick = kk == k ? H[k] : pick;
    return lane_read(pick, src);
}

template <int NCH, typename QF, typename TF>
__device__ int wave_ksw_global2_band(int qlen_, QF qf, int tlen_, TF tf, const slx_opt &o, int w_, uint8_t *z, int n_col_, int lane)
{
    const int qlen = __builtin_amdgcn_readfirstlane(qlen_), tlen = __builtin_amdgcn_readfirstlane(tlen_);
    const int w = __builtin_amdgcn_readfirstlane(w_), n_col = __builtin_amdgcn_readfirstlane(n_col_);
    const int o_del = o.o_del, e_del = o.e_del, o_ins = o.o_ins, e_ins = o.e_ins;
    const int oe_del = o_del + e_del, oe_ins = o_ins + e_ins;
    const MatCols mc = make_matcols(o.mat);
    auto pack_of = [&](int j) -> uint32_t {
        const int q = j >= 0 && j < qlen ? qf(j) : 4;
        return q == 0 ? mc.c[0] : q == 1 ? mc.c[1] : q == 2 ? mc.c[2] : q == 3 ? mc.c[3] : mc.c[4];
    };
    uint32_t Pblk[NCH];
#pragma unroll
    for (int c = 0; c < NCH; ++c) Pblk[c] = pack_of(c * WAVE + lane);
    const int b = lane, bE = b * e_ins;
    uint32_t P = pack_of(b - w);
    int H, E = DEV_MINUS_INF;
    {
        const int j = b - w;
        H = j == 0 ? 0 : (j > 0 && j <= qlen && j <= w ? -(o_ins + e_ins * j) : DEV_MINUS_INF);
    }
    int tb_cur = lane < tlen ? tf(lane) : 0;
    int tb_next = WAVE + lane < tlen ? tf(WAVE + lane) : 0;
#ifdef CIG_NOUNROLL
#pragma unroll 1
#endif
    for (int i = 0; i < tlen; ++i) {
        if ((i & (WAVE - 1)) == 0 && i) { tb_cur = tb_next; tb_next = i + WAVE + lane < tlen ? tf(i + WAVE + lane) : 0; }
        const int t = lane_read(tb_cur, i & (WAVE - 1));
        const uint32_t sh = (uint32_t)t << 3;
        const int beg = i > w ? i - w : 0;
        const int end = i + w + 1 < qlen ? i + w + 1 : qlen;
        const int b_lo = beg - (i - w), b_hi = end - (i - w);
        const bool act = b >= b_lo && b < b_hi;
        const int s = __builtin_amdgcn_sbfe((int)P, sh, 8u);
        const int m = H + s;
        const int u = act ? m - oe_ins + bE : G_NEG;
        const int incl = dpp_incl_max_scan_g(u);
        const int ex = dpp_get<0x138, 0xf, 0xf>(G_NEG, incl);
        int f = DEV_MINUS_INF - (b - b_lo) * e_ins;
        if (b > b_lo) f = imax(f, ex - (b - 1) * e_ins);
        const int e = E;
        int d = m >= e ? 0 : 1;
        int hh = m >= e ? m : e;
        d = hh >= f ? d : 2;
        hh = hh >= f ? hh : f;
        int tt = m - oe_del;
        int e2 = e - e_del;
        d |= e2 > tt ? 1 << 2 : 0;
        e2 = e2 > tt ? e2 : tt;
        tt = m - oe_ins;
        const int f2 = f - e_ins;
        d |= f2 > tt ? 2 << 4 : 0;
        if (act && z) z[(size_t)i * n_col + (b - b_lo)] = (uint8_t)d;
        if (act) H = hh;
        if (b == w - (i + 1)) H = -(o_del + e_del * (i + 1));
        const int e_up = dpp_get<0x130, 0xf, 0xf>(DEV_MINUS_INF, act ? e2 : DEV_MINUS_INF);
        E = e_up;
        const int jn = i + 1 + w;
        uint32_t pin = Pblk[0];
#pragma unroll
        for (int c = 1; c < NCH; ++c) pin = (jn >> 6) == c ? Pblk[c] : pin;
        const uint32_t p_new = jn < qlen ? (uint32_t)lane_read((int)pin, jn & (WAVE - 1)) : mc.c[4];
        const uint32_t p_up = (uint32_t)dpp_get<0x130, 0xf, 0xf>(0, (int)P);
        P = b == 2 * w ? p_new : p_up;
    }
    return lane_read(H, qlen - 1 - (tlen - 1 - w));
}

template <int MAXQ>
struct WaveScorer {
    const DevRef &R; const slx_opt &o; const MatRows &mr; int lane;
    __device__ int operator()(int w_, int l_query, const uint8_t *qseg, int64_t rb, int64_t re) const
    {
        constexpr int CPLMAX = (MAXQ + 1 + WAVE - 1) / WAVE;
        if (l_query <= 0 || rb >= re || (rb < R.l_pac && re > R.l_pac)) return 0;
        const int rlen = (int)(re - rb);
        const bool rev = rb >= R.l_pac;
        auto qf = [&](int x) { return (int)(rev ? qseg[l_query - 1 - x] : qseg[x]); };
        auto tf = [&](int y) { return rev ? ref_base(R, re - 1 - y) : ref_base(R, rb + y); };
        if (l_query == rlen && w_ == 0) {
            int sc = 0;
            for (int i = 0; i < l_query; ++i) sc += o.mat[tf(i) * 5 + qf(i)];
            return sc;
        }
        int max_ins = (int)((double)(((l_query + 1) >> 1) * o.mat[0] - o.o_ins) / o.e_ins + 1.);
        int max_del = (int)((double)(((l_query + 1) >> 1) * o.mat[0] - o.o_del) / o.e_del + 1.);
        int max_gap = max_ins > max_del ? max_ins : max_del;
        max_gap = max_gap > 1 ? max_gap : 1;
        const int dl = rlen - l_query < 0 ? l_query - rlen : rlen - l_query;
        int w = (max_gap + dl + 1) >> 1;
        w = w < w_ ? w : w_;
        const int min_w = dl + 3;
        w = w > min_w ? w : min_w;
        if (l_query + 1 <= WAVE) return wave_ksw_global2<1>(l_query, qf, rlen, tf, o, mr, w, nullptr, 0, lane);
        if (CPLMAX > 2 && l_query + 1 <= 2 * WAVE) return wave_ksw_global2<(CPLMAX > 2 ? 2 : CPLMAX)>(l_query, qf, rlen, tf, o, mr, w, nullptr, 0, lane);
        return wave_ksw_global2<CPLMAX>(l_query, qf, rlen, tf, o, mr, w, nullptr, 0, lane);
    }
};

__device__ __forceinline__ bool dev_reg_emit(const Chunk &ck, const slx_opt &opt, const FinLists &fl, int r, uint64_t slot, const DReg &ar, bool leader)
{
    const bool drop_sec = !ck.sam_mode && (ck.keepSecFrac < 0.0 || ck.keepSecFrac > 1.0);
    if (ar.secondary != 0 && drop_sec) return false;
    DHit h;
    h.flag = ar.secondary >= 0 ? 0x100 : 0;
    h.mapq = ar.secondary < 0 ? dev_approx_mapq_se(opt, ar, ck) : 0;
    h.score = ar.score; h.nm = -1; h.n_cigar = 0; h.cig_start = 0; h.pos = 0; h.rid = -1;
    const int qb = ar.qb, qe = ar.qe;
    const int64_t rb = ar.rb, re = ar.re;
    int tmp = dev_infer_bw(qe - qb, (int)(re - rb), ar.truesc, opt.a, opt.o_del, opt.e_del);
    int w2 = dev_infer_bw(qe - qb, (int)(re - rb), ar.truesc, opt.a, opt.o_ins, opt.e_ins);
    w2 = w2 > tmp ? w2 : tmp;
    if (w2 > opt.w) w2 = w2 < ar.w ? w2 : ar.w;
    DJob j;
    j.rb = rb; j.re = re; j.qb = qb; j.qe = qe; j.w2 = w2; j.truesc = ar.truesc; j.r = r; j.pad = 0;
    ck.hits[slot] = h;
    fl.jobs[slot] = j;
    const int wc = w2 < opt.w << 2 ? w2 : opt.w << 2;
    const bool fast = (qe - qb) == (int)(re - rb) && wc == 0;
    if (leader) {
        bool lanes = false;
        if (!fast && fl.lane_list && qe - qb <= LANE_CIG_MAXQ) {
            const int lq = qe - qb, rlen = (int)(re - rb);
            const int max_ins = (int)((double)(((lq + 1) >> 1) * opt.mat[0] - opt.o_ins) / opt.e_ins + 1.);
            const int max_del = (int)((double)(((lq + 1) >> 1) * opt.mat[0] - opt.o_del) / opt.e_del + 1.);
            int max_gap = max_ins > max_del ? max_ins : max_del;
            max_gap = max_gap > 1 ? max_gap : 1;
            const int dl = rlen - lq < 0 ? lq - rlen : rlen - lq;
            int ww = (max_gap + dl + 1) >> 1;
            ww = ww < wc ? ww : wc;
            ww = ww > dl + 3 ? ww : dl + 3;
            lanes = 2 * ww + 1 <= LANE_CIG_BAND && lq > 0 && rlen > 0 && rlen <= LANE_CIG_MAXT;
        }
        if (fast) fl.fast_list[wave_fetch_inc(fl.n_fast)] = (uint32_t)slot;
        else if (lanes) fl.lane_list[wave_fetch_inc(fl.n_lane)] = (uint32_t)slot;
        else fl.dp_list[wave_fetch_inc(fl.n_dp)] = (uint32_t)slot;
    }
    return true;
}

template <int MAXQ, typename SC>
__device__ void dev_regs_read(const DevRef &R, const Chunk &ck, const slx_opt &opt, const FinLists &fl, int r, SC &sc, bool leader,
                              const SortStage *ss = nullptr, int *defer_list = nullptr, unsigned int *n_defer = nullptr)
{
    ReadWS w = make_ws(ck, r);
    const uint8_t *query = ck.codes + ck.offs[r];
    const int l_query = (int)(ck.offs[r + 1] - ck.offs[r]);
    bool deferred = false;
    const int n = dev_fin_regs<MAXQ>(R, ck, opt, w, r, query, l_query, sc, ss, defer_list ? &deferred : nullptr);
    if (deferred) { defer_list[atomicAdd(n_defer, 1u)] = r; return; }
    const int *a = w.ia;
    const DReg *G = w.regs;
    const uint64_t so = ck.seed_off[r];
    int nh = 0;
    if (ss) {
        const bool drop_sec = !ck.sam_mode && (ck.keepSecFrac < 0.0 || ck.keepSecFrac > 1.0);
        for (int base = 0; base < n; base += 64) {
            const int i = base + ss->lane;
            DReg ar;
            bool keep = false;
            if (i < n) { ar = G[a[i]]; keep = !(ar.secondary != 0 && drop_sec); }
            const unsigned long long km = __ballot(keep);
            const int pos = nh + (int)__builtin_amdgcn_mbcnt_hi((uint32_t)(km >> 32), __builtin_amdgcn_mbcnt_lo((uint32_t)km, 0u));
            if (keep) dev_reg_emit(ck, opt, fl, r, so + pos, ar, true);
            nh += (int)__popcll(km);
        }
        if (leader) ck.n_hit[r] = nh;
        return;
    }
    for (int i = 0; i < n; ++i)
        if (dev_reg_emit(ck, opt, fl, r, so + nh, G[a[i]], leader)) ++nh;
    if (leader) ck.n_hit[r] = nh;
}

__global__ void __launch_bounds__(256) k_regs1(Chunk ck, DevOpt dopt, FinLists fl, const int *list, const unsigned int *n_list)
{
    const slx_opt &opt = dopt.o;
    const unsigned int n = *n_list;
    for (unsigned int t = blockIdx.x * blockDim.x + threadIdx.x; t < n; t += gridDim.x * blockDim.x) {
        const int r = list ? list[t] : (int)t;
        const int nr = ck.n_reg[r];
        int nh = 0;
        if (nr > 0) {
            const uint64_t so = ck.seed_off[r];
            DReg ar = ck.regs[so];
            ar.sub = 0; ar.secondary = -1;
            if (ck.sam_mode) {
                ck.regs[so].sub = 0; ck.regs[so].secondary = -1;
                ck.ia[so] = 0;
                if (ar.score >= opt.T && dev_reg_emit(ck, opt, fl, r, so, ar, true)) { nh = 1; ck.hits[so].flag |= (int)0x80000000; }
            } else if (dev_reg_emit(ck, opt, fl, r, so, ar, true)) nh = 1;
            ck.ic[so] = 0;
        }
        ck.na[r] = nr > 0 ? 1 : 0;
        ck.n_hit[r] = nh;
    }
}

template <int MAXQ>
__global__ void __launch_bounds__(128) k_regs(DevRef R, Chunk ck, DevOpt dopt, FinLists fl, const int *order, unsigned int *queue, const unsigned int *n_slots, int per_wave,
                                              int big_regs = 0, int *defer_list = nullptr, unsigned int *n_defer = nullptr)
{
    const slx_opt &opt = dopt.o;
    constexpr bool LONG = MAXQ > 704;
    int eh_hl[LONG ? 1 : MAXQ + 2], eh_el[LONG ? 1 : MAXQ + 2];
    int *eh_h = eh_hl, *eh_e = eh_el;
    if (LONG) {
        const int tid = blockIdx.x * blockDim.x + threadIdx.x;
        if (tid >= ck.long_threads) return;
        eh_h = ck.long_scratch + (size_t)tid * 2 * ck.long_stride; eh_e = eh_h + ck.long_stride;
    }
    const int n_todo = (int)*n_slots;
    if (per_wave) __builtin_amdgcn_s_setprio(3);
    auto sc = [&](int band, int lq, const uint8_t *qseg, int64_t rb, int64_t re) {
        return dev_gen_cigar2<MAXQ>(R, opt, ck, band, lq, qseg, rb, re, false, eh_h, eh_e).score;
    };
    while (true) {
        const int slot = next_slot(queue, per_wave);
        if (__all(slot >= n_todo)) break;
        if (slot >= n_todo) continue;
        const int r = order ? order[slot] : slot;
        if (!(big_regs > 0 && ck.n_reg[r] >= big_regs)) dev_regs_read<MAXQ>(R, ck, opt, fl, r, sc, true, nullptr, defer_list, n_defer);
    }
}

template <int MAXQ>
__device__ __noinline__ void dev_regs_read_wave(const DevRef &R, const Chunk &ck, const slx_opt &opt, const MatRows &mr, const FinLists &fl, int r, int lane,
                                                const SortStage *ss)
{
    WaveScorer<MAXQ> sc{R, opt, mr, lane};
    dev_regs_read<MAXQ>(R, ck, opt, fl, r, sc, lane == 0, ss);
}

#define REGS_SMALL_N 64
#define REGS_BIG_N 2048
#ifndef REGS_MID_N
#define REGS_MID_N 640
#endif
template <int MAXQ, int NB>
__global__ void __launch_bounds__(64) k_regs_wave(DevRef R, Chunk ck, DevOpt dopt, FinLists fl, const int *order, unsigned int *queue, const unsigned int *n_slots,
                                                  int min_regs, int max_regs)
{
    __shared__ int s_idx[NB], s_ka[NB], s_kb[NB], s_qe[NB], s_rid[NB], s_w[NB];
    __shared__ int64_t s_k64[NB], s_rb[NB];
    const int lane = threadIdx.x;
    SortStage ss;
    ss.idx = s_idx; ss.k64 = s_k64; ss.ka = s_ka; ss.kb = s_kb; ss.m_rb = s_rb; ss.m_qe = s_qe; ss.m_rid = s_rid; ss.m_w = s_w;
    ss.nmax = NB; ss.lane = lane;
    const MatRows mr = make_matrows(dopt.o.mat);
    const int n_todo = __builtin_amdgcn_readfirstlane((int)*n_slots);
    for (;;) {
        const int slot = (int)wave_take(queue, 1u);
        if (slot >= n_todo) break;
        const int r = order ? order[slot] : slot;
        const int nr = __builtin_amdgcn_readfirstlane(ck.n_reg[r]);
        const bool mine = nr >= min_regs && nr <= max_regs;
        if (mine) dev_regs_read_wave<MAXQ>(R, ck, dopt.o, mr, fl, r, lane, &ss);
#ifdef REGS_SLEEP
        if (mine && nr >= 256) for (int t = 0; t < REGS_SLEEP; ++t) __builtin_amdgcn_s_sleep(127);
#endif
    }
}

__device__ __forceinline__ void dev_finish_hit(const DevRef &R, const Chunk &ck, const DJob &j, int l_query, DHit &h, int64_t cs, int nc)
{
    int is_rev;
    int64_t pos = dev_depos(R, j.rb < R.l_pac ? j.rb : j.re - 1, &is_rev);
    if (nc > 0) {
        if ((ck.cigpool[cs] & 0xf) == 2) { pos += ck.cigpool[cs] >> 4; ++cs; --nc; }
        else if ((ck.cigpool[cs + nc - 1] & 0xf) == 2) --nc;
    }
    if (j.qb != 0 || j.qe != l_query) {
        const int clip5 = is_rev ? l_query - j.qe : j.qb, clip3 = is_rev ? j.qb : l_query - j.qe;
        const uint32_t cop = ck.hardclip ? 5u : 4u;
        if (clip5) { --cs; ck.cigpool[cs] = (uint32_t)clip5 << 4 | cop; ++nc; }
        if (clip3) { ck.cigpool[cs + nc] = (uint32_t)clip3 << 4 | cop; ++nc; }
    }
    h.rid = dev_pos2rid(R, pos);
    h.pos = pos - R.ann_off[h.rid];
    if (is_rev) h.flag |= 0x10;
    h.n_cigar = nc; h.cig_start = cs;
}

__global__ void __launch_bounds__(256) k_cig_fast(DevRef R, Chunk ck, FinLists fl)
{
    const unsigned int n = *fl.n_fast;
    for (unsigned int t = blockIdx.x * blockDim.x + threadIdx.x; t < n; t += gridDim.x * blockDim.x) {
        const uint32_t slot = fl.fast_list[t];
        const DJob j = fl.jobs[slot];
        DHit h = ck.hits[slot];
        const uint8_t *query = ck.codes + ck.offs[j.r];
        const int l_query = (int)(ck.offs[j.r + 1] - ck.offs[j.r]);
        const int lq = j.qe - j.qb;
        typedef uint64_t __attribute__((aligned(1))) u64u;
        int nm = 0, i = 0;
        const uint8_t *qp = query + j.qb;
        const bool rev = j.rb >= R.l_pac;
        for (; i + 8 <= lq; i += 8) {
            const uint64_t qw = *(const u64u *)(qp + i);
            uint64_t rw = 0;
            if (!rev) {
                const int64_t p0 = j.rb + i;
                const uint64_t L = *(const u64u *)(R.pac + (p0 >> 2));
#pragma unroll
                for (int k = 0; k < 8; ++k) {
                    const int64_t pk = p0 + k;
                    const int sh = (int)(((pk >> 2) - (p0 >> 2)) << 3) + (int)((~pk & 3) << 1);
                    rw |= ((L >> sh) & 3ull) << (8 * k);
                }
            } else {
                const int64_t f0 = (R.l_pac << 1) - 1 - (j.rb + i);
                const int64_t fb = (f0 - 7) >> 2;
                const uint64_t L = *(const u64u *)(R.pac + fb);
#pragma unroll
                for (int k = 0; k < 8; ++k) {
                    const int64_t fk = f0 - k;
                    const int sh = (int)(((fk >> 2) - fb) << 3) + (int)((~fk & 3) << 1);
                    rw |= (3ull - ((L >> sh) & 3ull)) << (8 * k);
                }
            }
            uint64_t d = qw ^ rw;
            d |= d >> 4; d |= d >> 2; d |= d >> 1;
            nm += __popcll(d & 0x0101010101010101ull);
        }
        for (; i < lq; ++i) {
            const int qc = qp[i];
            nm += qc != ref_base(R, j.rb + i);
        }
        h.nm = nm;
        const unsigned long long base = wave_fetch_add_u64(ck.cigused, 3ull);
        if (base + 3 > ck.cigcap) { atomicOr(ck.flags, OVF_CIGAR | OVS_C_FAST); continue; }
        ck.cigpool[base + 1] = (uint32_t)lq << 4;
        dev_finish_hit(R, ck, j, l_query, h, (int64_t)base + 1, 1);
        ck.hits[slot] = h;
    }
}

__global__ void __launch_bounds__(256) k_cig_fast_coop(DevRef R, Chunk ck, FinLists fl)
{
    __shared__ uint64_t s_q[4][64];
    __shared__ int64_t s_rb[4][64];
    __shared__ int s_lq[4][64], s_nm[4][64];
    const unsigned int n = *fl.n_fast;
    const int lane = threadIdx.x & 63, wv = threadIdx.x >> 6;
    for (unsigned int base = (blockIdx.x * 4u + (unsigned int)wv) * 64u; base < n; base += gridDim.x * 256u) {
        const unsigned int t = base + (unsigned int)lane;
        const bool valid = t < n;
        uint32_t slot = 0;
        DJob j;
        j.rb = j.re = 0; j.qb = j.qe = 0; j.w2 = j.truesc = 0; j.r = 0; j.pad = 0;
        int l_query = 0;
        uint64_t q_at0 = 0;
        if (valid) {
            slot = fl.fast_list[t];
            j = fl.jobs[slot];
            const uint64_t o0 = ck.offs[j.r];
            l_query = (int)(ck.offs[j.r + 1] - o0);
            q_at0 = o0 + (uint64_t)j.qb;
        }
        const int lq = valid ? j.qe - j.qb : 0;
        s_q[wv][lane] = q_at0; s_rb[wv][lane] = j.rb; s_lq[wv][lane] = lq; s_nm[wv][lane] = 0;
        int nch = (lq + 7) >> 3;
        for (int d = 32; d >= 1; d >>= 1) { const int o = __shfl_xor(nch, d, 64); nch = nch > o ? nch : o; }
        nch = __builtin_amdgcn_readfirstlane(nch);
        __builtin_amdgcn_fence(__ATOMIC_RELEASE, "wavefront"); __builtin_amdgcn_wave_barrier(); __builtin_amdgcn_fence(__ATOMIC_ACQUIRE, "wavefront");
        if (nch > 0) {
            int jj = lane / nch, c = lane - jj * nch;
            const int dj = 64 / nch, dc = 64 - dj * nch;
            for (; jj < 64; ) {
                const int i = c << 3, lqj = s_lq[wv][jj];
                if (i < lqj) {
                    const int nv = lqj - i < 8 ? lqj - i : 8;
                    const int m = nm8_chunk(R.pac, R.l_pac, ck.codes + s_q[wv][jj] + (uint64_t)i, s_rb[wv][jj] + i, nv);
                    if (m) atomicAdd(&s_nm[wv][jj], m);
                }
                jj += dj; c += dc;
                if (c >= nch) { c -= nch; ++jj; }
            }
        }
        __builtin_amdgcn_fence(__ATOMIC_RELEASE, "wavefront"); __builtin_amdgcn_wave_barrier(); __builtin_amdgcn_fence(__ATOMIC_ACQUIRE, "wavefront");
        if (!valid) continue;
        DHit h = ck.hits[slot];
        h.nm = s_nm[wv][lane];
        const unsigned long long cbase = wave_fetch_add_u64(ck.cigused, 3ull);
        if (cbase + 3 > ck.cigcap) { atomicOr(ck.flags, OVF_CIGAR | OVS_C_FAST_COOP); continue; }
        ck.cigpool[cbase + 1] = (uint32_t)lq << 4;
        dev_finish_hit(R, ck, j, l_query, h, (int64_t)cbase + 1, 1);
        ck.hits[slot] = h;
    }
}

template <typename F>
__device__ void dev_traceback_wave(const uint8_t *z, int n_col, int qlen, int tlen, int w, int lane, F emit)
{
    int i = tlen - 1, k = (i + w + 1 < qlen ? i + w + 1 : qlen) - 1, which = 0;
    int cur_op = -1, cur_len = 0;
    auto unit = [&](int op, int len) {
        if (op == cur_op) cur_len += len;
        else { if (cur_op >= 0) emit(cur_op, cur_len); cur_op = op; cur_len = len; }
    };
    while (i >= 0 && k >= 0) {
        if (which == 0) {
            const int it = i - lane, kt = k - lane;
            int d = 1;
            if (it >= 0 && kt >= 0) d = z[(size_t)it * n_col + (kt - (it > w ? it - w : 0))] & 3;
            const unsigned long long stop = __ballot(d != 0);
            const int run = stop ? (int)__ffsll((long long)stop) - 1 : WAVE;
            if (run > 0) { unit(0, run); i -= run; k -= run; continue; }
        }
        which = z[(size_t)i * n_col + (k - (i > w ? i - w : 0))] >> (which << 1) & 3;
        if (which == 0) { unit(0, 1); --i; --k; }
        else if (which == 1) { unit(2, 1); --i; }
        else { unit(1, 1); --k; }
    }
    if (i >= 0) unit(2, i + 1);
    if (k >= 0) unit(1, k + 1);
    if (cur_op >= 0) emit(cur_op, cur_len);
}

struct CigWaveState {
    uint8_t *z_own; unsigned long long z_own_cap;
    unsigned long long cig_next, cig_end;
};
#define CIG_WAVE_Z (16u << 10)
#define CIG_WAVE_WORDS 256u
#define CIG_BATCH 4

template <int MAXQ>
static __device__ __noinline__ void dev_cig_dp_job(const DevRef &R, const Chunk &ck, const slx_opt &opt, const MatRows &mr, const FinLists &fl,
                                            uint32_t slot, int lane, CigWaveState &ws)
{
    constexpr int CPLMAX = (MAXQ + 1 + WAVE - 1) / WAVE;
    const DJob j = fl.jobs[slot];
    DHit h = ck.hits[slot];
    const uint8_t *query = ck.codes + ck.offs[j.r];
    const int l_query = (int)(ck.offs[j.r + 1] - ck.offs[j.r]);
    const int lq = j.qe - j.qb;
    const int64_t rb = j.rb, re = j.re;
    const uint8_t *qseg = query + j.qb;
    const bool valid = !(lq <= 0 || rb >= re || (rb < R.l_pac && re > R.l_pac));
    const int rlen = (int)(re - rb);
    const bool rev = rb >= R.l_pac;
    auto qf = [&](int x) { return (int)(rev ? qseg[lq - 1 - x] : qseg[x]); };
    auto tf = [&](int y) { return rev ? ref_base(R, re - 1 - y) : ref_base(R, rb + y); };
    int w2 = j.w2, score = 0, last_sc = -(1 << 30), w_used = 0, n_col = 0;
    uint8_t *z = nullptr;
    if (valid) {
        for (int it = 0; it < 3; ++it) {
            w2 = w2 < opt.w << 2 ? w2 : opt.w << 2;
            int ww, max_gap, max_ins, max_del, min_w;
            max_ins = (int)((double)(((lq + 1) >> 1) * opt.mat[0] - opt.o_ins) / opt.e_ins + 1.);
            max_del = (int)((double)(((lq + 1) >> 1) * opt.mat[0] - opt.o_del) / opt.e_del + 1.);
            max_gap = max_ins > max_del ? max_ins : max_del;
            max_gap = max_gap > 1 ? max_gap : 1;
            const int dl = rlen - lq < 0 ? lq - rlen : rlen - lq;
            ww = (max_gap + dl + 1) >> 1;
            ww = ww < w2 ? ww : w2;
            min_w = dl + 3;
            ww = ww > min_w ? ww : min_w;
            w_used = ww;
            n_col = lq < 2 * ww + 1 ? lq : 2 * ww + 1;
            const unsigned long long need = (unsigned long long)n_col * (unsigned long long)rlen;
            if (need <= ws.z_own_cap) z = ws.z_own;
            else {
                const unsigned long long off = wave_take_u64(ck.zused, need);
                if (off + need > ck.zcap) { if (lane == 0) atomicOr(ck.flags, OVF_ZARENA | OVS_Z_DP); return; }
                z = ck.zarena + off;
            }
            if (2 * ww + 1 <= WAVE && lq <= (MAXQ + 2 + WAVE - 1) / WAVE * WAVE)
                score = wave_ksw_global2_band<(MAXQ + 2 + WAVE - 1) / WAVE>(lq, qf, rlen, tf, opt, ww, z, n_col, lane);
            else if (lq + 1 <= WAVE) score = wave_ksw_global2<1>(lq, qf, rlen, tf, opt, mr, ww, z, n_col, lane);
            else if (CPLMAX > 2 && lq + 1 <= 2 * WAVE) score = wave_ksw_global2<(CPLMAX > 2 ? 2 : CPLMAX)>(lq, qf, rlen, tf, opt, mr, ww, z, n_col, lane);
            else score = wave_ksw_global2<CPLMAX>(lq, qf, rlen, tf, opt, mr, ww, z, n_col, lane);
            if (score == last_sc || w2 == opt.w << 2) break;
            last_sc = score;
            w2 <<= 1;
            if (!(score < j.truesc - opt.a)) break;
        }
    }
    int n_ops = 0;
    if (valid) {
        __threadfence();
        dev_traceback_wave(z, n_col, lq, rlen, w_used, lane, [&](int, int) { ++n_ops; });
    }
    n_ops = __builtin_amdgcn_readfirstlane(n_ops);
    unsigned long long base = 0;
    const unsigned long long need = (unsigned long long)n_ops + 2;
    if (ws.cig_next + need > ws.cig_end) {
        const unsigned long long take = need > CIG_WAVE_WORDS ? need : (unsigned long long)CIG_WAVE_WORDS;
        base = wave_take_u64(ck.cigused, take);
        if (base + take > ck.cigcap) { if (lane == 0) atomicOr(ck.flags, OVF_CIGAR | OVS_C_DP); return; }
        ws.cig_next = base; ws.cig_end = base + take;
    }
    base = ws.cig_next; ws.cig_next += need;
    uint32_t *cg = ck.cigpool + base + 1;
    if (valid) {
        int wp = n_ops;
        dev_traceback_wave(z, n_col, lq, rlen, w_used, lane, [&](int op, int len) { cg[--wp] = (uint32_t)len << 4 | (uint32_t)op; });
        int x = 0, y = 0, n_mm = 0, n_gap = 0;
        for (int k = 0; k < n_ops; ++k) {
            const uint32_t cw = cg[k];
            const int op = (int)(cw & 0xf), len = (int)(cw >> 4);
            if (op == 0) {
                for (int u = lane; u < len; u += WAVE) n_mm += qf(x + u) != tf(y + u);
                x += len; y += len;
            } else if (op == 2) { if (k > 0 && k < n_ops - 1) n_gap += len; y += len; }
            else if (op == 1) { x += len; n_gap += len; }
        }
        for (int d = 32; d >= 1; d >>= 1) n_mm += __shfl_xor(n_mm, d, WAVE);
        h.nm = n_mm + n_gap;
    }
    dev_finish_hit(R, ck, j, l_query, h, (int64_t)base + 1, n_ops);
    if (lane == 0) ck.hits[slot] = h;
}

#ifndef CIG_MIN_WAVES
#define CIG_MIN_WAVES 4
#endif
template <int MAXQ>
__global__ void __launch_bounds__(64, CIG_MIN_WAVES) k_cig_dp(DevRef R, Chunk ck, DevOpt dopt, FinLists fl, int hi_prio)
{
    const int lane = threadIdx.x;
    if (hi_prio) __builtin_amdgcn_s_setprio(3);
    const MatRows mr = make_matrows(dopt.o.mat);
    const unsigned int n_jobs = *fl.n_dp;
    if (n_jobs == 0) return;
    CigWaveState ws;
    ws.z_own = nullptr; ws.z_own_cap = 0; ws.cig_next = ws.cig_end = 0;
    if (blockIdx.x < (n_jobs + CIG_BATCH - 1) / CIG_BATCH) {
        const unsigned long long off = wave_take_u64(ck.zused, (unsigned long long)CIG_WAVE_Z);
        if (off + CIG_WAVE_Z <= ck.zcap) { ws.z_own = ck.zarena + off; ws.z_own_cap = CIG_WAVE_Z; }
        else if (lane == 0) atomicOr(ck.flags + 1, OVS_Z_DP_WAVE);
    }
    for (;;) {
        const unsigned int t0 = wave_take(fl.q_dp, (unsigned int)CIG_BATCH);
        if (t0 >= n_jobs) break;
        const unsigned int t1 = t0 + CIG_BATCH < n_jobs ? t0 + CIG_BATCH : n_jobs;
        for (unsigned int t = t0; t < t1; ++t) dev_cig_dp_job<MAXQ>(R, ck, dopt.o, mr, fl, fl.dp_list[t], lane, ws);
    }
}

#define HITS_BIG 12
#define HITS_WAVE_N 2048
__global__ void __launch_bounds__(64) k_hits_wave(Chunk ck, const int *list, const unsigned int *n_list, unsigned int *queue)
{
    __shared__ int64_t s_pos[HITS_WAVE_N];
    __shared__ int s_rid[HITS_WAVE_N], s_mapq[HITS_WAVE_N];
    const int lane = threadIdx.x;
    const int n_todo = __builtin_amdgcn_readfirstlane((int)*n_list);
    for (;;) {
        const int slot = (int)wave_take(queue, 1u);
        if (slot >= n_todo) break;
        const int r = list[slot];
        ReadWS w = make_ws(ck, r);
        const int nh = __builtin_amdgcn_readfirstlane(ck.n_hit[r]);
        int *hh = w.ic;
        auto less_glb = [&](int x, int y) {
            const DHit &A = w.hits[x], &B = w.hits[y];
            if (A.mapq != B.mapq) return A.mapq > B.mapq;
            if (A.rid != B.rid) return A.rid < B.rid;
            return A.pos < B.pos;
        };
        bool serial = nh > HITS_WAVE_N;
        if (!serial) {
            __syncthreads();
            for (int e = lane; e < nh; e += 64) { const DHit &h = w.hits[e]; s_pos[e] = h.pos; s_rid[e] = h.rid; s_mapq[e] = h.mapq; }
            __syncthreads();
            bool tie = false;
            for (int base = 0; base < nh; base += 64) {
                const int e = base + lane;
                const bool live = e < nh;
                const int em = live ? s_mapq[e] : 0, er = live ? s_rid[e] : 0;
                const int64_t ep = live ? s_pos[e] : 0;
                int rank = 0;
                for (int j = 0; j < nh; ++j) {
                    const int jm = s_mapq[j], jr = s_rid[j];
                    const int64_t jp = s_pos[j];
                    const bool lt = jm != em ? jm > em : (jr != er ? jr < er : jp < ep);
                    rank += lt ? 1 : 0;
                    if (live && j != e && jm == em && jr == er && jp == ep) tie = true;
                }
                if (live) hh[rank] = e;
            }
            serial = __any(tie) != 0;
        }
        __threadfence_block();
        if (serial) {
            if (lane == 0) {
                for (int i = 0; i < nh; ++i) hh[i] = i;
                std_sort_idx(nh, hh, less_glb);
            }
            __threadfence_block();
        }
        __syncthreads();
        int n_out = 0;
        double carry = 0;
        for (int base = 0; base < nh; base += 64) {
            const int i = base + lane;
            const bool live = i < nh;
            const int hi = live ? hh[i] : 0;
            int flag = 0, score = 0;
            if (live) { const DHit &h = w.hits[hi]; flag = h.flag; score = h.score; }
            const bool isSec = live && (flag & 0x100) != 0;
            const unsigned long long prim = __ballot(live && !isSec);
            const unsigned long long below = prim & ((1ULL << lane) - 1ULL);
            const int src = below ? 63 - (int)__clzll((long long)below) : 0;
            const int sc_src = __shfl(score, src, 64);
            const double primaryScore = below ? (double)sc_src : carry;
            const bool tooLow = isSec && (primaryScore * ck.keepSecFrac > (double)score);
            const bool tooMany = isSec && (i > ck.maxSecondary);
            const bool keep = live && !(tooLow || tooMany);
            const unsigned long long km = __ballot(keep);
            const int pos = n_out + (int)__builtin_amdgcn_mbcnt_hi((uint32_t)(km >> 32), __builtin_amdgcn_mbcnt_lo((uint32_t)km, 0u));
            __syncthreads();
            if (keep) hh[pos] = hi;
            n_out += (int)__popcll(km);
            if (prim) { const int last = 63 - (int)__clzll((long long)prim); carry = (double)__shfl(score, last, 64); }
        }
        if (lane == 0) ck.n_hit[r] = n_out;
    }
}

__global__ void __launch_bounds__(128) k_hits(Chunk ck, const int *order, unsigned int *queue, const unsigned int *n_slots, int per_wave, int *big_list = nullptr,
                                              unsigned int *n_big = nullptr)
{
    const int n_todo = (int)*n_slots;
    if (per_wave) __builtin_amdgcn_s_setprio(3);
    while (true) {
        const int slot = next_slot(queue, per_wave);
        if (__all(slot >= n_todo)) break;
        if (slot >= n_todo) continue;
        const int r = order ? order[slot] : slot;
        ReadWS w = make_ws(ck, r);
        const int nh = ck.n_hit[r];
        if (big_list && nh > HITS_BIG) big_list[atomicAdd(n_big, 1u)] = r;
        else {
            int *hh = w.ic;
            for (int i = 0; i < nh; ++i) hh[i] = i;
            std_sort_idx(nh, hh, [&](int x, int y) {
                const DHit &A = w.hits[x], &B = w.hits[y];
                if (A.mapq != B.mapq) return A.mapq > B.mapq;
                if (A.rid != B.rid) return A.rid < B.rid;
                return A.pos < B.pos;
            });
            double primaryScore = 0;
            int n_out = 0;
            for (int i = 0; i < nh; ++i) {
                const DHit &h = w.hits[hh[i]];
                const bool isSec = (h.flag & 0x100) != 0;
                const bool tooLow = isSec && (primaryScore * ck.keepSecFrac > (double)h.score);
                const bool tooMany = isSec && (i > ck.maxSecondary);
                if (tooLow || tooMany) continue;
                if (!isSec) primaryScore = (double)h.score;
                hh[n_out++] = hh[i];
            }
            ck.n_hit[r] = n_out;
        }
    }
}

__global__ void __launch_bounds__(128) k_hits_sam(DevRef R, Chunk ck, DevOpt dopt, const int *order, unsigned int *queue, const unsigned int *n_slots)
{
    const slx_opt &opt = dopt.o;
    const int n_todo = (int)*n_slots;
    while (true) {
        const int slot = next_slot(queue, 0);
        if (__all(slot >= n_todo)) break;
        if (slot >= n_todo) continue;
        const int r = order ? order[slot] : slot;
        ReadWS w = make_ws(ck, r);
        const int n = ck.n_hit[r];
        const int *a = w.ia;
        const DReg *G = w.regs;
        int *hh = w.ic, *cnt = w.ib;
        int *rec_of = (int *)w.srt + w.cap;
        const int *sec_all = (const int *)w.srt;
        auto pri_of = [&](int i) {
            const int k = R.ann_alt ? sec_all[a[i]] : G[a[i]].secondary;
            if (k >= 0 && (double)G[a[i]].score >= (double)G[a[k]].score * (double)opt.XA_drop_ratio) return k;
            return -1;
        };
        for (int i = 0; i < n; ++i) cnt[i] = 0;
        for (int i = 0; i < n; ++i) {
            const int p = pri_of(i);
            if (p >= 0) cnt[p] = (cnt[p] + 1) | (ref_is_alt(R, G[a[i]].rid) ? 1 << 30 : 0);
        }
        int n_rec = 0, first_mapq = 0;
        for (int k = 0; k < n; ++k) {
            const DReg &p = G[a[k]];
            rec_of[k] = -1;
            if (p.score < opt.T || p.secondary >= 0) continue;
            DHit &h = w.hits[k];
            if (n_rec) {
                h.flag |= 0x800;
                if (!ref_is_alt(R, p.rid) && h.mapq > first_mapq) h.mapq = first_mapq;
            } else first_mapq = h.mapq;
            rec_of[k] = n_rec++;
        }
        if (n_rec > 0x7ffe) atomicOr(ck.flags, ERR_INTERNAL);
        int n_out = 0;
        for (int i = 0; i < n; ++i) {
            int par = -1;
            const int p = pri_of(i);
            if (p >= 0) {
                const int c = cnt[p] & 0x3fffffff;
                const bool listed = !(c > opt.max_XA_hits_alt || (!(cnt[p] >> 30) && c > opt.max_XA_hits));
                if (listed && rec_of[p] >= 0) par = rec_of[p];
            }
            if (rec_of[i] < 0 && par < 0) continue;
            w.hits[i].flag = (w.hits[i].flag & 0xffff) | ((par + 1) & 0x7fff) << 16 | (rec_of[i] >= 0 ? (int)0x80000000 : 0);
            hh[n_out++] = i;
        }
        ck.n_hit[r] = n_out;
    }
}
```

Baseline: 74.41 million.

## Use explicit LDS/global address spaces and wave-uniform scalars in chain and finish kernels

Shared-memory tables become typed LDS address-space pointers packed into structs, and workspace pointers are cast to global address space. Option fields, l_pac and base pointers are made wave-uniform through readfirstlane. The goal is to stop the compiler emitting generic flat loads and stores and to let uniform values sit in scalar registers in the noinline chaining and region-finishing routines. A manual s_waitcnt is added after a global load on the tree path, which could serialise memory traffic.

```diff
diff --git a/seqlib_amd/csrc/dev_as.h b/seqlib_amd/csrc/dev_as.h
--- /dev/null
+++ b/seqlib_amd/csrc/dev_as.h
@@ -0,0 +1,30 @@
+#pragma once
+#include <hip/hip_runtime.h>
+#include <stdint.h>
+#include "dev_wave.h"
+
+template <typename T> using lds_ptr = __attribute__((address_space(3))) T *;
+template <typename T> using glb_ptr = __attribute__((address_space(1))) T *;
+
+template <typename T> __device__ __forceinline__ glb_ptr<T> as_glb(T *p) { return (glb_ptr<T>)p; }
+template <typename T> __device__ __forceinline__ lds_ptr<T> as_lds(T *p) { return (lds_ptr<T>)p; }
+template <typename T> __device__ __forceinline__ glb_ptr<T> as_glb_uniform(T *p) { return (glb_ptr<T>)rfl_u64((uint64_t)p); }
+template <typename T> __device__ __forceinline__ T glb_load(glb_ptr<const T> p)
+{
+    static_assert(sizeof(T) % 8 == 0 && alignof(T) >= 8, "glb_load: a record of 8-byte words");
+    T v;
+    uint64_t *d = (uint64_t *)&v;
+    const glb_ptr<const uint64_t> s = (glb_ptr<const uint64_t>)p;
+#pragma unroll
+    for (int k = 0; k < (int)(sizeof(T) / 8); ++k) d[k] = s[k];
+    return v;
+}
+
+template <typename T> __device__ __forceinline__ lds_ptr<T> lds_uniform(lds_ptr<T> p)
+{
+    return (lds_ptr<T>)(uintptr_t)(uint32_t)__builtin_amdgcn_readfirstlane((int)(uint32_t)(uintptr_t)p);
+}
+
+__device__ __forceinline__ int rfl_i32(int v) { return __builtin_amdgcn_readfirstlane(v); }
+__device__ __forceinline__ float rfl_f32(float v) { return __int_as_float(__builtin_amdgcn_readfirstlane(__float_as_int(v))); }
+__device__ __forceinline__ int64_t rfl_i64(int64_t v) { return (int64_t)rfl_u64((uint64_t)v); }
diff --git a/seqlib_amd/csrc/dev_chain_coop.h b/seqlib_amd/csrc/dev_chain_coop.h
--- a/seqlib_amd/csrc/dev_chain_coop.h
+++ b/seqlib_amd/csrc/dev_chain_coop.h
@@ -1,5 +1,6 @@
 #pragma once
 #include "dev_chain.h"
+#include "dev_as.h"
 
 __device__ __forceinline__ int64_t lane_read64(int64_t v, int src)
 {
@@ -9,21 +10,41 @@
     return (int64_t)(((unsigned long long)hi << 32) | lo);
 }
 
+template <int NCMAX>
 struct CoopTables {
-    int64_t *s_pos;
-    int *s_ord;
-    int *s_w, *s_cb, *s_ce, *s_first, *s_kept;
-    signed char *s_kf;
+    int64_t pos[NCMAX + 64];
+    int ord[NCMAX + 64];
+    int w[NCMAX], cb[NCMAX], ce[NCMAX], first[NCMAX], kept[NCMAX];
+    signed char kf[NCMAX];
 };
 
+struct CoopWS {
+    glb_ptr<int64_t> s_rbeg; glb_ptr<qp_t> s_ql; glb_ptr<int32_t> s_next, s_score;
+    glb_ptr<int64_t> c_pos; glb_ptr<int32_t> c_head, c_tail, c_n, c_rid, c_w, c_first, ia;
+    __device__ __forceinline__ int s_qbeg(int s) const { return QP_HI(s_ql[s]); }
+    __device__ __forceinline__ int s_len(int s) const { return QP_LO(s_ql[s]); }
+};
+
 template <typename I, int NCMAX, bool FINAL>
-__device__ __noinline__ void dev_chain_read_coop(const DevFM<I> &fm, const DevRef &R, const Chunk &ck, const slx_opt &opt, int r, const CoopTables &T, int lane,
-                                                 int nc_limit)
+__device__ __noinline__ void dev_chain_read_coop(const DevFM<I> &fm, const DevRef &R, const Chunk &ck, const slx_opt &opt, int r_, lds_ptr<CoopTables<NCMAX>> T, int lane,
+                                                 int nc_limit_)
 {
-    int64_t *s_pos = T.s_pos; int *s_ord = T.s_ord, *s_w = T.s_w, *s_cb = T.s_cb, *s_ce = T.s_ce, *s_first = T.s_first, *s_kept = T.s_kept;
-    signed char *s_kf = T.s_kf;
+    const int r = rfl_i32(r_), nc_limit = rfl_i32(nc_limit_);
+    const lds_ptr<int64_t> s_pos = T->pos;
+    const lds_ptr<int> s_ord = T->ord, s_w = T->w, s_cb = T->cb, s_ce = T->ce, s_first = T->first, s_kept = T->kept;
+    const lds_ptr<signed char> s_kf = T->kf;
+    const int o_w = rfl_i32(opt.w), o_max_chain_gap = rfl_i32(opt.max_chain_gap), o_max_occ = rfl_i32(opt.max_occ);
+    const int o_min_chain_weight = rfl_i32(opt.min_chain_weight), o_min_seed_len = rfl_i32(opt.min_seed_len), o_max_chain_extend = rfl_i32(opt.max_chain_extend);
+    const float o_mask_level = rfl_f32(opt.mask_level), o_drop_ratio = rfl_f32(opt.drop_ratio);
+    const int64_t l_pac = rfl_i64(R.l_pac);
+    const glb_ptr<const uint8_t> ann_alt = as_glb_uniform(R.ann_alt);
+    auto is_alt = [&](int rid) { return ann_alt && rid >= 0 ? (int)ann_alt[rid] : 0; };
     {
-        ReadWS w = make_ws(ck, r);
+        const ReadWS w0 = make_ws(ck, r);
+        CoopWS w;
+        w.s_rbeg = as_glb_uniform(w0.s_rbeg); w.s_ql = as_glb_uniform(w0.s_ql); w.s_next = as_glb_uniform(w0.s_next); w.s_score = as_glb_uniform(w0.s_score);
+        w.c_pos = as_glb_uniform(w0.c_pos); w.c_head = as_glb_uniform(w0.c_head); w.c_tail = as_glb_uniform(w0.c_tail); w.c_n = as_glb_uniform(w0.c_n);
+        w.c_rid = as_glb_uniform(w0.c_rid); w.c_w = as_glb_uniform(w0.c_w); w.c_first = as_glb_uniform(w0.c_first); w.ia = as_glb_uniform(w0.ia);
         const int len = (int)(ck.offs[r + 1] - ck.offs[r]);
         const int n_intv = (int)ck.intv_n[r];
         const qp_t *iinfo = (const qp_t *)ck.intv_info + (size_t)r * ck.cap_intv;
@@ -33,14 +54,14 @@
         bool dup = false;
         KbTree kb;
         bool tree = false;
-        int *l_tail = s_w, *l_lastql = s_cb, *l_lastoff = s_ce, *l_firstql = s_first, *l_rid = s_kept;
+        const lds_ptr<int> l_tail = s_w, l_lastql = s_cb, l_lastoff = s_ce, l_firstql = s_first, l_rid = s_kept;
         const bool cnt16 = ck.seed_off[r + 1] - ck.seed_off[r] < 65536;
         for (int i = 0; i < n_intv; ++i) {
             const int qbeg = QP_HI(iinfo[i]), slen = QP_LO(iinfo[i]) - qbeg;
             const I x0 = ix0[i], x2 = ix2[i];
-            const I step = x2 > (I)opt.max_occ ? x2 / (I)opt.max_occ : (I)1;
+            const I step = x2 > (I)o_max_occ ? x2 / (I)o_max_occ : (I)1;
             I cm = (x2 + step - 1) / step;
-            if (cm > (I)opt.max_occ) cm = (I)opt.max_occ;
+            if (cm > (I)o_max_occ) cm = (I)o_max_occ;
             const int count_max = (int)cm;
             for (int base = 0; base < count_max; base += 64) {
                 const int t = base + lane;
@@ -77,16 +98,20 @@
                             const int f_qbeg = (int)(fql >> 16);
 #endif
                             const int l_qbeg = QP_HI(lql), l_len = QP_LO(lql);
-                            const int64_t f_rbeg = tree ? w.c_pos[c] : s_pos[lo];
+                            int64_t f_rbeg;
+                            if (tree) {
+                                f_rbeg = w.c_pos[c];
+                                __builtin_amdgcn_s_waitcnt(0x0f70);
+                            } else f_rbeg = s_pos[lo];
                             const int64_t l_rbeg = f_rbeg + l_lastoff[c];
                             const int64_t qend = l_qbeg + l_len, rend = l_rbeg + l_len;
                             int res;
                             if (rid != l_rid[c]) res = 0;
                             else if (qbeg >= f_qbeg && qbeg + slen <= qend && rbeg >= f_rbeg && rbeg + slen <= rend) res = 1;
-                            else if ((l_rbeg < R.l_pac || f_rbeg < R.l_pac) && rbeg >= R.l_pac) res = 0;
+                            else if ((l_rbeg < l_pac || f_rbeg < l_pac) && rbeg >= l_pac) res = 0;
                             else {
                                 const int64_t x = qbeg - l_qbeg, y = rbeg - l_rbeg;
-                                if (y >= 0 && x - y <= opt.w && y - x <= opt.w && x - l_len < opt.max_chain_gap && y - l_len < opt.max_chain_gap) {
+                                if (y >= 0 && x - y <= o_w && y - x <= o_w && x - l_len < o_max_chain_gap && y - l_len < o_max_chain_gap) {
                                     const int s = ns++;
                                     w.s_rbeg[s] = rbeg; w.s_ql[s] = QP_PACK(qbeg, slen); w.s_next[s] = -1; if (w.s_score) w.s_score[s] = slen;
                                     w.s_next[last] = s; w.c_tail[c] = s;
@@ -106,7 +131,7 @@
                     }
                     if (to_add && !tree && lo >= 0 && s_pos[lo] == rbeg) dup = true;
                     if (to_add && dup && !tree && nc >= 2 * KB_T - 1) {
-                        kb.mem = (int *)w.regs; kb.n_nodes = 0; kb.root = kb.alloc(0);
+                        kb.mem = (int *)w0.regs; kb.n_nodes = 0; kb.root = kb.alloc(0);
                         for (int h = 0; h < nc; ++h) kb.put(w.c_pos[h], h);
                         tree = true;
                     }
@@ -140,7 +165,7 @@
                 }
             }
         }
-        if (tree) kb.traverse(s_ord);
+        if (tree) kb.traverse((int *)s_ord);
         ck.frac_rep[r] = (float)ck.l_rep[r] / len;
         for (int c = lane; c < nc; c += 64) {
             const int wt = dev_chain_weight(w, c);
@@ -153,7 +178,7 @@
         for (int base = 0; base < nc; base += 64) {
             const int m = base + lane;
             int c = 0; bool keep = false;
-            if (m < nc) { c = s_ord[m]; keep = s_w[c] >= opt.min_chain_weight; }
+            if (m < nc) { c = s_ord[m]; keep = s_w[c] >= o_min_chain_weight; }
             const unsigned long long bal = __ballot(keep);
             const int rank = __popcll(bal & ((1ull << lane) - 1ull));
             if (keep) s_ord[n_chn + rank] = c;
@@ -161,7 +186,7 @@
         }
         int n_out = 0;
         if (n_chn > 0) {
-            int *a = s_ord;
+            const lds_ptr<int> a = s_ord;
             ks_introsort_idx(n_chn, a, [&](int x, int y) { return s_w[x] > s_w[y]; });
             int n_kept = 0;
             s_kf[a[0]] = 3;
@@ -169,7 +194,7 @@
             for (int i = 1; i < n_chn; ++i) {
                 const int ci = a[i];
                 const int bi = s_cb[ci], ei = s_ce[ci], wi = s_w[ci], li = ei - bi;
-                const bool i_alt = ref_is_alt(R, w.c_rid[ci]) != 0;
+                const bool i_alt = is_alt(w.c_rid[ci]) != 0;
                 int large_ovlp = 0;
                 bool broke = false;
                 for (int kb = 0; kb < n_kept && !broke; kb += 64) {
@@ -180,13 +205,13 @@
                         cj = a[s_kept[k]];
                         const int bj = s_cb[cj], ej = s_ce[cj];
                         const int b_max = bj > bi ? bj : bi, e_min = ej < ei ? ej : ei;
-                        if (e_min > b_max && (!ref_is_alt(R, w.c_rid[cj]) || i_alt)) {
+                        if (e_min > b_max && (!is_alt(w.c_rid[cj]) || i_alt)) {
                             const int lj = ej - bj;
                             const int min_l = li < lj ? li : lj;
-                            if ((float)(e_min - b_max) >= (float)min_l * opt.mask_level && min_l < opt.max_chain_gap) {
+                            if ((float)(e_min - b_max) >= (float)min_l * o_mask_level && min_l < o_max_chain_gap) {
                                 large = true;
                                 const int wj = s_w[cj];
-                                if ((float)wi < (float)wj * opt.drop_ratio && wj - wi >= opt.min_seed_len << 1) drop = true;
+                                if ((float)wi < (float)wj * o_drop_ratio && wj - wi >= o_min_seed_len << 1) drop = true;
                             }
                         }
                     }
@@ -207,7 +232,7 @@
             for (i = k = 0; i < n_chn; ++i) {
                 const int kf = s_kf[a[i]];
                 if (kf == 0 || kf == 3) continue;
-                if (++k >= opt.max_chain_extend) break;
+                if (++k >= o_max_chain_extend) break;
             }
             for (int m = i + lane; m < n_chn; m += 64) if (s_kf[a[m]] < 3) s_kf[a[m]] = 0;
             for (int base = 0; base < n_chn; base += 64) {
@@ -244,12 +269,8 @@
 __global__ void __launch_bounds__(64) k_chain_coop(DevFM<I> fm, DevRef R, Chunk ck, DevOpt dopt, const int *order, unsigned int *queue,
                                                    const unsigned int *n_slots, int nc_limit)
 {
-    __shared__ int64_t s_pos[NCMAX + 64];
-    __shared__ int s_ord[NCMAX + 64];
-    __shared__ int s_w[NCMAX], s_cb[NCMAX], s_ce[NCMAX], s_first[NCMAX], s_kept[NCMAX];
-    __shared__ signed char s_kf[NCMAX];
-    CoopTables T;
-    T.s_pos = s_pos; T.s_ord = s_ord; T.s_w = s_w; T.s_cb = s_cb; T.s_ce = s_ce; T.s_first = s_first; T.s_kept = s_kept; T.s_kf = s_kf;
+    __shared__ CoopTables<NCMAX> tables;
+    const lds_ptr<CoopTables<NCMAX>> T = as_lds(&tables);
     const int lane = threadIdx.x;
     const int n_todo = __builtin_amdgcn_readfirstlane((int)*n_slots);
     for (;;) {
diff --git a/seqlib_amd/csrc/dev_cig_band.h b/seqlib_amd/csrc/dev_cig_band.h
--- a/seqlib_amd/csrc/dev_cig_band.h
+++ b/seqlib_amd/csrc/dev_cig_band.h
@@ -441,8 +441,7 @@
 __global__ void __launch_bounds__(GB_THREADS) k_regs_wave_long(DevRef R, Chunk ck, DevOpt dopt, FinLists fl, const int *order, unsigned int *queue, const unsigned int *n_slots,
                                                                PMemo pm)
 {
-    __shared__ int s_idx[NB], s_ka[NB], s_kb[NB], s_qe[NB], s_rid[NB], s_w[NB];
-    __shared__ int64_t s_k64[NB], s_rb[NB];
+    __shared__ SortTables<NB> tables;
     __shared__ RegsBlockShared SB;
     if ((int)blockIdx.x * WAVE >= ck.long_threads) return;
     if (threadIdx.x >= WAVE) {
@@ -454,9 +453,7 @@
         return;
     }
     const int lane = threadIdx.x;
-    SortStage ss;
-    ss.idx = s_idx; ss.k64 = s_k64; ss.ka = s_ka; ss.kb = s_kb; ss.m_rb = s_rb; ss.m_qe = s_qe; ss.m_rid = s_rid; ss.m_w = s_w;
-    ss.nmax = NB; ss.lane = lane;
+    const SortStage ss = tables.stage(lane);
     int *eh_h = ck.long_scratch + (size_t)blockIdx.x * WAVE * 2 * ck.long_stride, *eh_e = eh_h + ck.long_stride;
     int cur_r = 0;
     WaveScorerLong sc{R, dopt.o, ck, lane, eh_h, eh_e, &SB, pm.jobs ? &pm : nullptr, &cur_r};
diff --git a/seqlib_amd/csrc/dev_fin.h b/seqlib_amd/csrc/dev_fin.h
--- a/seqlib_amd/csrc/dev_fin.h
+++ b/seqlib_amd/csrc/dev_fin.h
@@ -1,5 +1,6 @@
 #pragma once
 #include "dev_ext.h"
+#include "dev_as.h"
 
 #define DEV_MINUS_INF (-0x40000000)
 
@@ -123,23 +124,28 @@
     return g;
 }
 
-__device__ __forceinline__ int dev_patch_pre(const DevRef &R, const slx_opt &o, int64_t a_rb, int64_t a_re, int a_qb, int a_qe, int a_w,
+__device__ __forceinline__ int dev_patch_pre(int64_t l_pac, int o_w, int64_t a_rb, int64_t a_re, int a_qb, int a_qe, int a_w,
                                              int64_t b_rb, int64_t b_re, int b_qb, int b_qe, int b_w)
 {
     int w;
     double r;
-    if (a_rb < R.l_pac && b_rb >= R.l_pac) return -1;
+    if (a_rb < l_pac && b_rb >= l_pac) return -1;
     if (a_qb >= b_qb || a_qe >= b_qe || a_re >= b_re) return -1;
     w = (int)((a_re - b_rb) - (a_qe - b_qb));
     w = w > 0 ? w : -w;
     r = (double)(a_re - b_rb) / (double)(b_re - a_rb) - (double)(a_qe - b_qb) / (double)(b_qe - a_qb);
     r = r > 0. ? r : -r;
     if (a_re < b_rb || a_qe < b_qb) {
-        if (w > o.w << 1 || r >= (double)0.05f) return -1;
-    } else if (w > o.w << 2 || r >= (double)(0.05f * 2)) return -1;
+        if (w > o_w << 1 || r >= (double)0.05f) return -1;
+    } else if (w > o_w << 2 || r >= (double)(0.05f * 2)) return -1;
     w += a_w + b_w;
-    w = w < o.w << 2 ? w : o.w << 2;
+    w = w < o_w << 2 ? w : o_w << 2;
     return w;
+}
+__device__ __forceinline__ int dev_patch_pre(const DevRef &R, const slx_opt &o, int64_t a_rb, int64_t a_re, int a_qb, int a_qe, int a_w,
+                                             int64_t b_rb, int64_t b_re, int b_qb, int b_qe, int b_w)
+{
+    return dev_patch_pre(R.l_pac, o.w, a_rb, a_re, a_qb, a_qe, a_w, b_rb, b_re, b_qb, b_qe, b_w);
 }
 
 template <int MAXQ, typename SC>
@@ -290,14 +296,26 @@
 }
 
 struct SortStage {
-    int *idx;
-    int64_t *k64;
-    int *ka, *kb;
-    int64_t *m_rb;
-    int *m_qe, *m_rid, *m_w;
+    lds_ptr<int> idx;
+    lds_ptr<int64_t> k64;
+    lds_ptr<int> ka, kb;
+    lds_ptr<int64_t> m_rb;
+    lds_ptr<int> m_qe, m_rid, m_w;
     int nmax;
     int lane;
 };
+template <int NB>
+struct SortTables {
+    int64_t k64[NB], rb[NB];
+    int idx[NB], ka[NB], kb[NB], qe[NB], rid[NB], w[NB];
+    __device__ __forceinline__ SortStage stage(int lane)
+    {
+        SortStage ss;
+        ss.idx = as_lds(idx); ss.k64 = as_lds(k64); ss.ka = as_lds(ka); ss.kb = as_lds(kb); ss.m_rb = as_lds(rb); ss.m_qe = as_lds(qe); ss.m_rid = as_lds(rid); ss.m_w = as_lds(w);
+        ss.nmax = NB; ss.lane = lane;
+        return ss;
+    }
+};
 
 template <int MAXQ>
 __device__ __forceinline__ void fin_sync()
@@ -313,45 +331,59 @@
         int n = ck.n_reg[r];
         int *a = w.ia;
         DReg *G = w.regs;
-        const bool staged = ss != nullptr && n <= ss->nmax && n >= 2;
+        const int o_max_chain_gap = rfl_i32(opt.max_chain_gap), o_w = rfl_i32(opt.w);
+        const float o_mask_level_redun = rfl_f32(opt.mask_level_redun), o_mask_level = rfl_f32(opt.mask_level);
+        const int64_t l_pac = rfl_i64(R.l_pac);
+        SortStage S;
+        S.idx = S.ka = S.kb = S.m_qe = S.m_rid = S.m_w = nullptr; S.k64 = S.m_rb = nullptr; S.nmax = 0; S.lane = 0;
+        if (ss) {
+            S.idx = lds_uniform(ss->idx); S.k64 = lds_uniform(ss->k64); S.ka = lds_uniform(ss->ka); S.kb = lds_uniform(ss->kb);
+            S.m_rb = lds_uniform(ss->m_rb); S.m_qe = lds_uniform(ss->m_qe); S.m_rid = lds_uniform(ss->m_rid); S.m_w = lds_uniform(ss->m_w);
+            S.nmax = rfl_i32(ss->nmax); S.lane = ss->lane;
+            n = rfl_i32(n);
+        }
+        const bool staged = ss != nullptr && n <= S.nmax && n >= 2;
+        glb_ptr<DReg> Gg = as_glb(G);
+        glb_ptr<int> ag = as_glb(a);
+        if (staged) { Gg = as_glb_uniform(G); ag = as_glb_uniform(a); }
         const bool dbg = ck.dbg_cyc && ck.dbg_stage == 2;
         unsigned long long t0 = dbg ? __builtin_readcyclecounter() : 0ull, t1 = t0, t2 = t0, t3 = t0;
         auto sort_handles = [&](int m, auto fill, auto less_lds, auto less_glb) {
             if (!staged) { ks_introsort_idx(m, a, less_glb); return; }
             __threadfence_block();
-            for (int i = ss->lane; i < m; i += 64) { const int h = a[i]; ss->idx[i] = h; fill(h); }
+            for (int i = S.lane; i < m; i += 64) { const int h = ag[i]; S.idx[i] = h; fill(h); }
             fin_sync<MAXQ>();
             bool tie = m > 768;
-            if (!tie) for (int e = ss->lane; e < m; e += 64) {
-                const int he = ss->idx[e];
+            if (!tie) for (int e = S.lane; e < m; e += 64) {
+                const int he = S.idx[e];
                 int rank = 0;
                 for (int j = 0; j < m; ++j) {
-                    const int hj = ss->idx[j];
+                    const int hj = S.idx[j];
                     const bool lt = less_lds(hj, he);
                     rank += lt ? 1 : 0;
                     if (!lt && j != e && !less_lds(he, hj)) tie = true;
                 }
-                ss->m_w[e] = rank;
+                S.m_w[e] = rank;
             }
             if (!__any(tie)) {
                 fin_sync<MAXQ>();
-                for (int e = ss->lane; e < m; e += 64) ss->m_rid[ss->m_w[e]] = ss->idx[e];
-                fin_sync<MAXQ>();
-                for (int e = ss->lane; e < m; e += 64) { const int h = ss->m_rid[e]; ss->idx[e] = h; a[e] = h; }
+                for (int e = S.lane; e < m; e += 64) S.m_rid[S.m_w[e]] = S.idx[e];
+                fin_sync<MAXQ>();
+                for (int e = S.lane; e < m; e += 64) { const int h = S.m_rid[e]; S.idx[e] = h; ag[e] = h; }
             } else {
                 fin_sync<MAXQ>();
-                if (ss->lane == 0) ks_introsort_idx(m, ss->idx, less_lds);
-                fin_sync<MAXQ>();
-                for (int i = ss->lane; i < m; i += 64) a[i] = ss->idx[i];
+                if (S.lane == 0) ks_introsort_idx(m, S.idx, less_lds);
+                fin_sync<MAXQ>();
+                for (int i = S.lane; i < m; i += 64) ag[i] = S.idx[i];
             }
             fin_sync<MAXQ>();
             __threadfence_block();
         };
-        if (staged) { for (int i = ss->lane; i < n; i += 64) a[i] = i; __threadfence_block(); }
+        if (staged) { for (int i = S.lane; i < n; i += 64) ag[i] = i; __threadfence_block(); }
         else for (int i = 0; i < n; ++i) a[i] = i;
         if (n > 1) {
-            sort_handles(n, [&](int h) { ss->k64[h] = G[h].re; },
-                         [&](int x, int y) { return ss->k64[x] < ss->k64[y]; },
+            sort_handles(n, [&](int h) { S.k64[h] = Gg[h].re; },
+                         [&](int x, int y) { return S.k64[x] < S.k64[y]; },
                          [&](int x, int y) { return G[x].re < G[y].re; });
             if (dbg) t1 = __builtin_readcyclecounter();
             if (defer && !staged && n <= 64) {
@@ -364,29 +396,32 @@
                     }
                 }
             }
-            if (staged) { for (int i = ss->lane; i < n; i += 64) G[i].n_comp = 1; __threadfence_block(); }
+            if (staged) { for (int i = S.lane; i < n; i += 64) Gg[i].n_comp = 1; __threadfence_block(); }
             else for (int i = 0; i < n; ++i) G[a[i]].n_comp = 1;
             if (staged) {
-                const int lane = ss->lane;
-                int64_t *m_re = ss->k64; int *m_sc = ss->ka, *m_qb = ss->kb;
+                const int lane = S.lane;
+                const lds_ptr<int64_t> m_re = S.k64; const lds_ptr<int> m_sc = S.ka, m_qb = S.kb;
                 for (int h = lane; h < n; h += 64) {
-                    const DReg &g = G[h];
-                    ss->m_rb[h] = g.rb; m_re[h] = g.re; m_qb[h] = g.qb; ss->m_qe[h] = g.qe; ss->m_rid[h] = g.rid; m_sc[h] = g.score; ss->m_w[h] = g.w;
+                    const glb_ptr<const DReg> g = Gg + h;
+                    S.m_rb[h] = g->rb; m_re[h] = g->re; m_qb[h] = g->qb; S.m_qe[h] = g->qe; S.m_rid[h] = g->rid; m_sc[h] = g->score; S.m_w[h] = g->w;
                 }
                 fin_sync<MAXQ>();
                 for (int i = 1; i < n; ++i) {
-                    const int ph = ss->idx[i], prevh = ss->idx[i - 1];
-                    if (ss->m_rid[ph] != ss->m_rid[prevh] || ss->m_rb[ph] >= m_re[prevh] + opt.max_chain_gap) continue;
+                    const int ph = S.idx[i], prevh = S.idx[i - 1];
+                    int64_t p_rb = S.m_rb[ph];
+                    const int p_rid = S.m_rid[ph];
+                    if (p_rid != S.m_rid[prevh] || p_rb >= m_re[prevh] + o_max_chain_gap) continue;
+                    const int64_t p_re = m_re[ph];
+                    const int p_qe = S.m_qe[ph];
+                    int p_qb = m_qb[ph], p_sc = m_sc[ph], p_w = S.m_w[ph];
                     int jtop = i - 1;
                     while (jtop >= 0) {
-                        const int64_t p_rb = ss->m_rb[ph], p_re = m_re[ph];
-                        const int p_qb = m_qb[ph], p_qe = ss->m_qe[ph], p_rid = ss->m_rid[ph], p_sc = m_sc[ph], p_w = ss->m_w[ph];
                         const int j = jtop - lane;
                         const bool valid = j >= 0;
-                        const int qh = ss->idx[valid ? j : 0];
-                        const int64_t q_rb = ss->m_rb[qh], q_re = m_re[qh];
-                        const int q_qb = m_qb[qh], q_qe = ss->m_qe[qh], q_sc = m_sc[qh], q_w = ss->m_w[qh];
-                        const bool cond = valid && p_rid == ss->m_rid[qh] && p_rb < q_re + opt.max_chain_gap;
+                        const int qh = S.idx[valid ? j : 0];
+                        const int64_t q_rb = S.m_rb[qh], q_re = m_re[qh];
+                        const int q_qb = m_qb[qh], q_qe = S.m_qe[qh], q_sc = m_sc[qh], q_w = S.m_w[qh];
+                        const bool cond = valid && p_rid == S.m_rid[qh] && p_rb < q_re + o_max_chain_gap;
                         const unsigned long long stopm = __ballot(!cond);
                         const int first_stop = stopm ? (int)__ffsll((long long)stopm) - 1 : 64;
                         const bool live = lane < first_stop;
@@ -396,12 +431,12 @@
                             const int64_t oq = q_qb < p_qb ? q_qe - p_qb : p_qe - q_qb;
                             const int64_t mr = q_re - q_rb < p_re - p_rb ? q_re - q_rb : p_re - p_rb;
                             const int64_t mq = q_qe - q_qb < p_qe - p_qb ? q_qe - q_qb : p_qe - p_qb;
-                            if ((float)orr > opt.mask_level_redun * (float)mr && (float)oq > opt.mask_level_redun * (float)mq) cat = p_sc < q_sc ? 2 : 1;
-                            else if (q_rb < p_rb && dev_patch_pre(R, opt, q_rb, q_re, q_qb, q_qe, q_w, p_rb, p_re, p_qb, p_qe, p_w) >= 0) cat = 3;
+                            if ((float)orr > o_mask_level_redun * (float)mr && (float)oq > o_mask_level_redun * (float)mq) cat = p_sc < q_sc ? 2 : 1;
+                            else if (q_rb < p_rb && dev_patch_pre(l_pac, o_w, q_rb, q_re, q_qb, q_qe, q_w, p_rb, p_re, p_qb, p_qe, p_w) >= 0) cat = 3;
                         }
                         const unsigned long long evm = __ballot(cat >= 2);
                         const int first_ev = evm ? (int)__ffsll((long long)evm) - 1 : 64;
-                        if (cat == 1 && lane < first_ev) { ss->m_qe[qh] = q_qb; G[qh].qe = q_qb; }
+                        if (cat == 1 && lane < first_ev) S.m_qe[qh] = q_qb;
                         fin_sync<MAXQ>();
                         if (first_ev == 64) {
                             if (first_stop < 64) break;
@@ -411,7 +446,7 @@
                         const int ev_cat = __builtin_amdgcn_readlane(cat, first_ev);
                         const int ev_q = __builtin_amdgcn_readlane(qh, first_ev);
                         if (ev_cat == 2) {
-                            if (lane == 0) { ss->m_qe[ph] = p_qb; G[ph].qe = p_qb; }
+                            if (lane == 0) S.m_qe[ph] = p_qb;
                             fin_sync<MAXQ>();
                             break;
                         }
@@ -430,15 +465,17 @@
                                 pp.w = ww;
                                 q.qb = q.qe;
                                 if (lane == 0) {
-                                    m_qb[ph] = m_qb[ev_q]; ss->m_rb[ph] = ss->m_rb[ev_q]; m_sc[ph] = score; ss->m_w[ph] = ww;
-                                    m_qb[ev_q] = ss->m_qe[ev_q];
+                                    m_qb[ph] = m_qb[ev_q]; S.m_rb[ph] = S.m_rb[ev_q]; m_sc[ph] = score; S.m_w[ph] = ww;
+                                    m_qb[ev_q] = S.m_qe[ev_q];
                                 }
                                 fin_sync<MAXQ>();
+                                p_rb = S.m_rb[ph]; p_qb = m_qb[ph]; p_sc = m_sc[ph]; p_w = S.m_w[ph];
                             }
                         }
                         jtop -= first_ev + 1;
                     }
                 }
+                for (int h = lane; h < n; h += 64) Gg[h].qe = S.m_qe[h];
                 __threadfence_block();
             } else
             for (int i = 1; i < n; ++i) {
@@ -472,12 +509,12 @@
             auto compact_staged = [&](int n_in, int first_forced) {
                 int m = 0;
                 for (int base = 0; base < n_in; base += 64) {
-                    const int i = base + ss->lane;
-                    const int h = i < n_in ? ss->idx[i] : 0;
-                    const bool keep = i < n_in && (i < first_forced || ss->m_qe[h] > ss->kb[h]);
+                    const int i = base + S.lane;
+                    const int h = i < n_in ? S.idx[i] : 0;
+                    const bool keep = i < n_in && (i < first_forced || S.m_qe[h] > S.kb[h]);
                     const unsigned long long km = __ballot(keep);
                     const int pos = m + (int)__builtin_amdgcn_mbcnt_hi((uint32_t)(km >> 32), __builtin_amdgcn_mbcnt_lo((uint32_t)km, 0u));
-                    if (keep) a[pos] = h;
+                    if (keep) ag[pos] = h;
                     m += (int)__popcll(km);
                 }
                 __threadfence_block();
@@ -487,20 +524,20 @@
             if (staged) m = compact_staged(n, 0);
             else for (int i = 0; i < n; ++i) if (G[a[i]].qe > G[a[i]].qb) a[m++] = a[i];
             n = m;
-            sort_handles(n, [&](int h) { ss->ka[h] = G[h].score; ss->k64[h] = G[h].rb; ss->kb[h] = G[h].qb; },
+            sort_handles(n, [&](int h) { S.ka[h] = Gg[h].score; S.k64[h] = Gg[h].rb; S.kb[h] = Gg[h].qb; },
                          [&](int x, int y) {
-                             const int sx = ss->ka[x], sy = ss->ka[y];
-                             const int64_t bx = ss->k64[x], by = ss->k64[y];
-                             return sx > sy || (sx == sy && (bx < by || (bx == by && ss->kb[x] < ss->kb[y])));
+                             const int sx = S.ka[x], sy = S.ka[y];
+                             const int64_t bx = S.k64[x], by = S.k64[y];
+                             return sx > sy || (sx == sy && (bx < by || (bx == by && S.kb[x] < S.kb[y])));
                          },
                          [&](int x, int y) {
                              const DReg &X = G[x], &Y = G[y];
                              return X.score > Y.score || (X.score == Y.score && (X.rb < Y.rb || (X.rb == Y.rb && X.qb < Y.qb)));
                          });
             if (staged) {
-                for (int i = 1 + ss->lane; i < n; i += 64) {
-                    const int h = ss->idx[i], hp = ss->idx[i - 1];
-                    if (ss->ka[h] == ss->ka[hp] && ss->k64[h] == ss->k64[hp] && ss->kb[h] == ss->kb[hp]) { G[h].qe = ss->kb[h]; ss->m_qe[h] = ss->kb[h]; }
+                for (int i = 1 + S.lane; i < n; i += 64) {
+                    const int h = S.idx[i], hp = S.idx[i - 1];
+                    if (S.ka[h] == S.ka[hp] && S.k64[h] == S.k64[hp] && S.kb[h] == S.kb[hp]) { Gg[h].qe = S.kb[h]; S.m_qe[h] = S.kb[h]; }
                 }
                 fin_sync<MAXQ>();
                 n = compact_staged(n, 1);
@@ -520,29 +557,29 @@
             int tmp = opt.a + opt.b;
             tmp = opt.o_del + opt.e_del > tmp ? opt.o_del + opt.e_del : tmp;
             tmp = opt.o_ins + opt.e_ins > tmp ? opt.o_ins + opt.e_ins : tmp;
-            auto core_staged = [&](int m, const int *l_alt) {
-                const int lane = ss->lane;
-                int *l_sub = ss->m_rid, *l_subn = ss->m_w, *l_sec = (int *)ss->k64, *l_z = (int *)ss->k64 + ss->nmax;
-                fin_sync<MAXQ>();
-                for (int i = lane; i < m; i += 64) { const int h = ss->idx[i]; l_sub[h] = 0; l_subn[h] = G[h].sub_n; l_sec[h] = -1; }
+            auto core_staged = [&](int m, lds_ptr<const int> l_alt) {
+                const int lane = S.lane;
+                const lds_ptr<int> l_sub = S.m_rid, l_subn = S.m_w, l_sec = (lds_ptr<int>)S.k64, l_z = (lds_ptr<int>)S.k64 + S.nmax;
+                fin_sync<MAXQ>();
+                for (int i = lane; i < m; i += 64) { const int h = S.idx[i]; l_sub[h] = 0; l_subn[h] = Gg[h].sub_n; l_sec[h] = -1; }
                 if (lane == 0) l_z[0] = 0;
                 fin_sync<MAXQ>();
                 int nz = 1;
                 for (int i = 1; i < m; ++i) {
-                    const int hi = ss->idx[i];
-                    const int i_qb = ss->kb[hi], i_qe = ss->m_qe[hi], i_sc = ss->ka[hi];
+                    const int hi = S.idx[i];
+                    const int i_qb = S.kb[hi], i_qe = S.m_qe[hi], i_sc = S.ka[hi];
                     int found = -1;
                     for (int kb0 = 0; kb0 < nz && found < 0; kb0 += 64) {
                         const int k = kb0 + lane;
                         bool hit = false;
                         if (k < nz) {
-                            const int hj = ss->idx[l_z[k]];
-                            const int j_qb = ss->kb[hj], j_qe = ss->m_qe[hj];
+                            const int hj = S.idx[l_z[k]];
+                            const int j_qb = S.kb[hj], j_qe = S.m_qe[hj];
                             const int b_max = j_qb > i_qb ? j_qb : i_qb;
                             const int e_min = j_qe < i_qe ? j_qe : i_qe;
                             if (e_min > b_max) {
                                 const int min_l = i_qe - i_qb < j_qe - j_qb ? i_qe - i_qb : j_qe - j_qb;
-                                hit = (float)(e_min - b_max) >= (float)min_l * opt.mask_level;
+                                hit = (float)(e_min - b_max) >= (float)min_l * o_mask_level;
                             }
                         }
                         const unsigned long long hm = __ballot(hit);
@@ -551,65 +588,66 @@
                     if (found >= 0) {
                         if (lane == 0) {
                             const int zi = l_z[found];
-                            const int hj = ss->idx[zi];
+                            const int hj = S.idx[zi];
                             if (l_sub[hj] == 0) l_sub[hj] = i_sc;
-                            if (ss->ka[hj] - i_sc <= tmp && (!l_alt || l_alt[hj] || !l_alt[hi])) ++l_subn[hj];
+                            if (S.ka[hj] - i_sc <= tmp && (!l_alt || l_alt[hj] || !l_alt[hi])) ++l_subn[hj];
                             l_sec[hi] = zi;
                         }
                     } else { if (lane == 0) l_z[nz] = i; ++nz; }
                     fin_sync<MAXQ>();
                 }
-                for (int i = lane; i < m; i += 64) { const int h = ss->idx[i]; DReg &p = G[h]; p.sub = l_sub[h]; p.sub_n = l_subn[h]; p.secondary = l_sec[h]; }
+                for (int i = lane; i < m; i += 64) { const int h = S.idx[i]; const glb_ptr<DReg> p = Gg + h; p->sub = l_sub[h]; p->sub_n = l_subn[h]; p->secondary = l_sec[h]; }
                 __threadfence_block();
                 fin_sync<MAXQ>();
             };
             if (R.ann_alt && staged) {
-                const int lane = ss->lane;
-                int *l_alt = (int *)ss->m_rb, *l_par = (int *)ss->m_rb + ss->nmax, *par = (int *)w.srt;
+                const int lane = S.lane;
+                const lds_ptr<int> l_alt = (lds_ptr<int>)S.m_rb, l_par = (lds_ptr<int>)S.m_rb + S.nmax;
+                const glb_ptr<int> par = as_glb_uniform((int *)w.srt);
                 fin_sync<MAXQ>();
                 int n_pri = 0;
                 for (int base = 0; base < n; base += 64) {
                     const int i = base + lane;
                     bool pri = false;
                     if (i < n) {
-                        const int h = a[i];
-                        DReg &p = G[h];
-                        p.sub = 0; p.secondary = -1; p.hash = dev_hash_64(id + (uint64_t)i);
-                        const int al = ref_is_alt(R, p.rid);
+                        const int h = ag[i];
+                        const glb_ptr<DReg> p = Gg + h;
+                        p->sub = 0; p->secondary = -1; p->hash = dev_hash_64(id + (uint64_t)i);
+                        const int al = ref_is_alt(R, p->rid);
                         l_alt[h] = al;
                         pri = !al;
                     }
                     n_pri += (int)__popcll(__ballot(pri));
                 }
                 __threadfence_block();
-                sort_handles(n, [&](int h) { ss->ka[h] = G[h].score; ss->k64[h] = (int64_t)G[h].hash; },
+                sort_handles(n, [&](int h) { S.ka[h] = Gg[h].score; S.k64[h] = (int64_t)Gg[h].hash; },
                              [&](int x, int y) {
-                                 const int sx = ss->ka[x], sy = ss->ka[y];
+                                 const int sx = S.ka[x], sy = S.ka[y];
                                  if (sx != sy) return sx > sy;
                                  const int ax = l_alt[x], ay = l_alt[y];
-                                 return ax < ay || (ax == ay && (uint64_t)ss->k64[x] < (uint64_t)ss->k64[y]);
+                                 return ax < ay || (ax == ay && (uint64_t)S.k64[x] < (uint64_t)S.k64[y]);
                              },
                              [&](int x, int y) { return false; });
                 core_staged(n, l_alt);
                 if (n_pri < n) {
-                    for (int i = lane; i < n; i += 64) { const int h = ss->idx[i], sidx = G[h].secondary; l_par[h] = sidx >= 0 ? ss->idx[sidx] : -1; }
+                    for (int i = lane; i < n; i += 64) { const int h = S.idx[i], sidx = Gg[h].secondary; l_par[h] = sidx >= 0 ? S.idx[sidx] : -1; }
                     fin_sync<MAXQ>();
                     if (n_pri > 0)
-                        sort_handles(n, [&](int h) { ss->ka[h] = G[h].score; ss->k64[h] = (int64_t)G[h].hash; },
+                        sort_handles(n, [&](int h) { S.ka[h] = Gg[h].score; S.k64[h] = (int64_t)Gg[h].hash; },
                                      [&](int x, int y) {
                                          const int ax = l_alt[x], ay = l_alt[y];
                                          if (ax != ay) return ax < ay;
-                                         const int sx = ss->ka[x], sy = ss->ka[y];
-                                         return sx > sy || (sx == sy && (uint64_t)ss->k64[x] < (uint64_t)ss->k64[y]);
+                                         const int sx = S.ka[x], sy = S.ka[y];
+                                         return sx > sy || (sx == sy && (uint64_t)S.k64[x] < (uint64_t)S.k64[y]);
                                      },
                                      [&](int x, int y) { return false; });
-                    int *l_rank = (int *)ss->k64;
+                    const lds_ptr<int> l_rank = (lds_ptr<int>)S.k64;
                     fin_sync<MAXQ>();
-                    for (int i = lane; i < n; i += 64) l_rank[ss->idx[i]] = i;
+                    for (int i = lane; i < n; i += 64) l_rank[S.idx[i]] = i;
                     fin_sync<MAXQ>();
                     for (int i = lane; i < n; i += 64) {
-                        const int h = ss->idx[i], ph = l_par[h];
-                        if (ph >= 0) { par[h] = l_rank[ph]; if (l_alt[h]) G[h].secondary = 0x7fffffff; }
+                        const int h = S.idx[i], ph = l_par[h];
+                        if (ph >= 0) { par[h] = l_rank[ph]; if (l_alt[h]) Gg[h].secondary = 0x7fffffff; }
                         else par[h] = -1;
                     }
                     if (n_pri > 0) {
@@ -617,24 +655,24 @@
                         core_staged(n_pri, l_alt);
                     }
                 } else
-                    for (int i = lane; i < n; i += 64) { const int h = ss->idx[i]; par[h] = G[h].secondary; }
+                    for (int i = lane; i < n; i += 64) { const int h = S.idx[i]; par[h] = Gg[h].secondary; }
                 __threadfence_block();
                 fin_sync<MAXQ>();
             } else if (R.ann_alt) {
                 dev_mark_primary_alt(R, opt, w, n, id);
             } else {
             if (staged) {
-                for (int i = ss->lane; i < n; i += 64) { DReg &p = G[a[i]]; p.sub = 0; p.secondary = -1; p.hash = dev_hash_64(id + (uint64_t)i); }
+                for (int i = S.lane; i < n; i += 64) { const glb_ptr<DReg> p = Gg + ag[i]; p->sub = 0; p->secondary = -1; p->hash = dev_hash_64(id + (uint64_t)i); }
                 __threadfence_block();
             } else for (int i = 0; i < n; ++i) {
                 DReg &p = G[a[i]];
                 p.sub = 0; p.secondary = -1;
                 p.hash = dev_hash_64(id + (uint64_t)i);
             }
-            sort_handles(n, [&](int h) { ss->ka[h] = G[h].score; ss->k64[h] = (int64_t)G[h].hash; },
+            sort_handles(n, [&](int h) { S.ka[h] = Gg[h].score; S.k64[h] = (int64_t)Gg[h].hash; },
                          [&](int x, int y) {
-                             const int sx = ss->ka[x], sy = ss->ka[y];
-                             return sx > sy || (sx == sy && (uint64_t)ss->k64[x] < (uint64_t)ss->k64[y]);
+                             const int sx = S.ka[x], sy = S.ka[y];
+                             return sx > sy || (sx == sy && (uint64_t)S.k64[x] < (uint64_t)S.k64[y]);
                          },
                          [&](int x, int y) {
                              const DReg &X = G[x], &Y = G[y];
diff --git a/seqlib_amd/csrc/dev_fin2.h b/seqlib_amd/csrc/dev_fin2.h
--- a/seqlib_amd/csrc/dev_fin2.h
+++ b/seqlib_amd/csrc/dev_fin2.h
@@ -283,11 +283,13 @@
     int nh = 0;
     if (ss) {
         const bool drop_sec = !ck.sam_mode && (ck.keepSecFrac < 0.0 || ck.keepSecFrac > 1.0);
+        const glb_ptr<const DReg> Gg = as_glb_uniform(G);
+        const glb_ptr<const int> ag = as_glb_uniform(a);
         for (int base = 0; base < n; base += 64) {
             const int i = base + ss->lane;
             DReg ar;
             bool keep = false;
-            if (i < n) { ar = G[a[i]]; keep = !(ar.secondary != 0 && drop_sec); }
+            if (i < n) { ar = glb_load<DReg>(Gg + ag[i]); keep = !(ar.secondary != 0 && drop_sec); }
             const unsigned long long km = __ballot(keep);
             const int pos = nh + (int)__builtin_amdgcn_mbcnt_hi((uint32_t)(km >> 32), __builtin_amdgcn_mbcnt_lo((uint32_t)km, 0u));
             if (keep) dev_reg_emit(ck, opt, fl, r, so + pos, ar, true);
@@ -369,12 +371,9 @@
 __global__ void __launch_bounds__(64) k_regs_wave(DevRef R, Chunk ck, DevOpt dopt, FinLists fl, const int *order, unsigned int *queue, const unsigned int *n_slots,
                                                   int min_regs, int max_regs)
 {
-    __shared__ int s_idx[NB], s_ka[NB], s_kb[NB], s_qe[NB], s_rid[NB], s_w[NB];
-    __shared__ int64_t s_k64[NB], s_rb[NB];
+    __shared__ SortTables<NB> tables;
     const int lane = threadIdx.x;
-    SortStage ss;
-    ss.idx = s_idx; ss.k64 = s_k64; ss.ka = s_ka; ss.kb = s_kb; ss.m_rb = s_rb; ss.m_qe = s_qe; ss.m_rid = s_rid; ss.m_w = s_w;
-    ss.nmax = NB; ss.lane = lane;
+    const SortStage ss = tables.stage(lane);
     const MatRows mr = make_matrows(dopt.o.mat);
     const int n_todo = __builtin_amdgcn_readfirstlane((int)*n_slots);
     for (;;) {
```

Result: faster. 77.92 million (median of 6 runs) (+4.7%).
